# LaurenYTaylor/jsrl-CORL

Measured on AMD Instinct MI355X. Metric: IQL gradient-steps/sec at batch=256 (D4RL obs/act dims), higher is better.
Workload: dtype f32; 1 GPU; IQL step on synthetic buffer (obs=17, act=6, 1000000 rows), batch=256 per GPU; global_batch=256, parallelism=single, prepare_rehearsal_steps=1111

## Files before the change

include/iqlhip.h:

```cpp
#ifndef IQLHIP_H
#define IQLHIP_H

#include <stdint.h>

#ifdef __cplusplus
extern "C" {
#endif

#define IQLHIP_VERSION 400
#define IQLHIP_HIDDEN 256
#define IQLHIP_MAX_INPUT 128
#define IQLHIP_MAX_ACTION 32
#define IQLHIP_MAX_WORLD 8
#define IQLHIP_GRAPH_STEPS 64
#define IQLHIP_N_SCORE 8
#define IQLHIP_N_STATS 16

enum {
  IQLHIP_OK = 0,
  IQLHIP_EINVAL = -1,
  IQLHIP_EHIP = -2,
  IQLHIP_ENOTBOUND = -3,
  IQLHIP_EUNSUPPORTED = -4,
  IQLHIP_EINDEX = -5,
// ... 241 lines not shown
                            void* stream);
int iqlhip_group_train_steps(iqlhip_group* group, const float* const* rows, int64_t ld, const int64_t* size, int32_t B,
                             const void* const* tables, int32_t n, const uint64_t* seeds, const uint64_t* offsets,
                             int32_t flags, void* stream);
int iqlhip_group_train_steps_mixed(iqlhip_group* group, const float* const* rows, int64_t ld, const int64_t* size,
                                   const int32_t* B, const void* const* tables, int32_t n, const uint64_t* seeds,
                                   const uint64_t* offsets, int32_t flags, void* stream);
int iqlhip_group_read_losses(iqlhip_group* group, float* out, int32_t n, void* stream);
int iqlhip_group_read_step_stats(iqlhip_group* group, float* out, int32_t n, void* stream);
int iqlhip_group_online_step(iqlhip_group* group, float* const* rows_dev, int64_t ld, const int64_t* capacity,
                             const int64_t* pointer, const float* row_host, const int64_t* idx_host, int32_t n,
                             const iqlhip_step_scalars* sc, float* out, const float* act_state_host,
                             const int32_t* act_mask, const float* max_action, const uint64_t* act_seed,
                             float* act_out_host, void* stream);
int iqlhip_group_online_step_mixed(iqlhip_group* group, float* const* rows_dev, int64_t ld, const int64_t* capacity,
                                   const int64_t* pointer, const float* row_host, const int64_t* idx_host,
                                   const int32_t* n, const iqlhip_step_scalars* sc, float* out,
                                   const float* act_state_host, const int32_t* act_mask, const float* max_action,
                                   const uint64_t* act_seed, float* act_out_host, void* stream);
int iqlhip_group_online_step_replay2(iqlhip_group* group, float* const* rows_dev, int64_t ld, const int64_t* capacity,
                                     const int64_t* pointer, const float* row_host, const int64_t* idx_host,
                                     const int32_t* n, const iqlhip_step_scalars* sc, float* out,
                                     const float* act_state_host, const int32_t* act_mask, const float* max_action,
                                     const uint64_t* act_seed, float* act_out_host, void* stream,
                                     const float* const* rows_off_dev, const int64_t* size_off, const int32_t* n_off);
int iqlhip_group_train_steps_replay2(iqlhip_group* group, const float* const* rows_off, const int64_t* size_off,
                                     const float* const* rows_on, const int64_t* size_on, int64_t ld, const int32_t* B,
                                     const int32_t* n_off, const void* const* tables, int32_t n, const uint64_t* seeds,
                                     const uint64_t* offsets, void* stream);
int iqlhip_group_train_steps_weighted(iqlhip_group* group, const float* const* rows, int64_t ld, const int64_t* size,
                                      const int32_t* B, const void* const* tables, int32_t n, const uint64_t* seeds,
                                      const uint64_t* offsets, int32_t flags, void* stream,
                                      const iqlhip_weights* const* wtabs);
#define IQLHIP_GROUP_TS_CONTINUE 1
int iqlhip_group_step_rw(iqlhip_group* group, const iqlhip_batch* batches, const iqlhip_step_scalars* sc,
                         const float* const* row_w_dev, float* const* td_out_dev, float* out, void* stream);
int iqlhip_group_train_steps_weighted_is(iqlhip_group* group, const float* const* rows, int64_t ld, const int64_t* size,
                                         const int32_t* B, const void* const* tables, int32_t n, const uint64_t* seeds,
                                         const uint64_t* offsets, int32_t flags, void* stream,
                                         const iqlhip_weights* const* wtabs, const float* is_beta);
int iqlhip_group_train_steps_prioritized(iqlhip_group* group, const float* const* rows, int64_t ld, const int64_t* size,
                                         const int32_t* B, const void* const* tables, int32_t n, const uint64_t* seeds,
                                         const uint64_t* offsets, int32_t flags, void* stream,
                                         iqlhip_weights* const* wtabs, const float* is_beta, const float* alpha,
                                         const float* eps);
#define IQLHIP_GROUP_ACT_WAIT 1
int iqlhip_group_actor_forward(iqlhip_group* group, const float* const* states, int64_t ld_s, const int32_t* rows,
                               const uint64_t* seeds, const float* max_action, float* const* actions, int64_t ld_a,
                               int32_t flags, void* stream);

int iqlhip_group_score_rows(iqlhip_group* group, const float* const* rows_dev, int64_t ld, const int64_t* n_rows,
                            int64_t row0, int64_t n, const int64_t* const* idx_dev, float* const* out_dev,
                            float* spread_dev, int32_t chunk_rows, float* summary , void* stream);

#define IQLHIP_ACT_ROWS 4096
int iqlhip_actor_forward(iqlhip_ctx* ctx, const float* states_dev, int64_t ld_s, int32_t rows, const float* noise_dev,
                         int64_t ld_noise, float max_action, float* actions_dev, int64_t ld_a, void* stream);

int iqlhip_actor_sample(iqlhip_ctx* ctx, const float* states_dev, int64_t ld_s, int32_t rows, uint64_t seed,
                        float max_action, float* actions_dev, int64_t ld_a, void* stream);

int iqlhip_stream_synchronize(void* stream);

typedef struct iqlhip_jsrl iqlhip_jsrl;
int iqlhip_jsrl_create(iqlhip_ctx* const* learners, iqlhip_ctx* const* guides, iqlhip_ctx* const* gates, int k,
                       iqlhip_jsrl** out);
int iqlhip_jsrl_destroy(iqlhip_jsrl* jsrl);
int iqlhip_jsrl_act(iqlhip_jsrl* jsrl, const float* const* states, int64_t ld_s, const int32_t* rows,
                    const int8_t* const* who, const float* gate_max, const uint64_t* seeds,
                    const float* max_action_learner, const float* max_action_guide, float* const* actions, int64_t ld_a,
                    int32_t* const* use_learner, float* const* gate_out, int32_t flags, void* stream);
int iqlhip_jsrl_online_step(iqlhip_jsrl* jsrl, float* rows_dev, int64_t ld, int64_t capacity, int64_t pointer,
                            const float* row_host, const int64_t* idx_host, int32_t n, const iqlhip_step_scalars* sc,
                            float out[3], const float* act_state_host, int8_t who, float gate_max, uint64_t act_seed,
                            float max_action_learner, float max_action_guide, float* act_out_host,
                            int32_t* use_learner_out, float* gate_out, void* stream);

int iqlhip_debug_read(iqlhip_ctx* ctx, const char* name, float* host_out, int64_t max_floats, int64_t* n_out,
                      void* stream);
int iqlhip_debug_time_kernel(iqlhip_ctx* ctx, const iqlhip_batch* batch, int which, int repeat, float* avg_us,
                             void* stream);
int iqlhip_debug_drain_spin(iqlhip_ctx* ctx, void* stream, double* spin_us);
int64_t iqlhip_debug_live_buffers(void);
int iqlhip_set_timing(iqlhip_ctx* ctx, int enabled);
int iqlhip_get_timing(iqlhip_ctx* ctx, float out_us[4]);

typedef struct iqlhip_var iqlhip_var;
typedef struct iqlhip_var_scalars {
  float step_size;
  float bc2_sqrt;
  float beta2, one_minus_beta1, one_minus_beta2, eps;
  int32_t aligned_rewards;
  int32_t reserved;
} iqlhip_var_scalars;
int iqlhip_var_layout(int32_t state_dim, iqlhip_net_layout out[2], int64_t* n_params);
int iqlhip_var_create(int32_t state_dim, int32_t max_rows, int device, iqlhip_var** out);
int iqlhip_var_destroy(iqlhip_var* var);
int iqlhip_var_bind(iqlhip_var* var, float* params, float* exp_avg, float* exp_avg_sq);
int iqlhip_var_step(iqlhip_var* var, const float* batch_dev, int32_t B, int32_t which_net, const iqlhip_var_scalars* sc,
                    void* stream);
int iqlhip_var_values(iqlhip_var* var, const float* batch_dev, int32_t B, int32_t aligned_rewards, float* out_dev,
                      void* stream);
int iqlhip_var_forward_backward(iqlhip_var* var, const float* batch_dev, int32_t B, int32_t which_net,
                                int32_t aligned_rewards, float* grad_out_dev, void* stream);
int iqlhip_var_read_loss(iqlhip_var* var, float* loss, float* head, int32_t n_head, void* stream);

#define IQLHIP_VAR_TRAIN_MAX_STEPS 1024
int iqlhip_var_pack_window(iqlhip_var* var, const float* rows_dev, int64_t ld, int64_t n_rows, int32_t state_dim,
                           int32_t action_dim, int64_t start, int32_t B, float* block_out_dev, void* stream);
int iqlhip_var_values_window(iqlhip_var* var, const float* rows_dev, int64_t ld, int64_t n_rows, int32_t state_dim,
                             int32_t action_dim, int64_t start, int32_t B, int32_t aligned_rewards, float* out_dev,
                             void* stream);
int iqlhip_var_train_steps(iqlhip_var* var, const float* rows_dev, int64_t ld, int64_t size, int32_t action_dim, int32_t B,
                           int32_t n_steps, int32_t which_net, const iqlhip_var_scalars* scalars, uint64_t seed,
                           uint64_t stream_offset, const int64_t* starts_dev, int64_t n_starts, void* stream);
int iqlhip_var_read_train_ring(iqlhip_var* var, float* losses_out, int64_t* starts_out, int32_t n_steps, void* stream);

typedef struct iqlhip_var_group iqlhip_var_group;
int iqlhip_var_group_create(iqlhip_var* const* members, int k, iqlhip_var_group** out);
int iqlhip_var_group_destroy(iqlhip_var_group* group);
int iqlhip_var_group_step(iqlhip_var_group* group, const float* const* blocks_dev, int32_t B, int32_t which_net,
                          const iqlhip_var_scalars* scalars, void* stream);
int iqlhip_var_group_values(iqlhip_var_group* group, const float* const* blocks_dev, int32_t B, const int32_t* aligned_rewards,
                            float* const* outs_dev, void* stream);
int iqlhip_var_group_read_loss(iqlhip_var_group* group, float* losses, float* heads, int32_t n_head, void* stream);
int iqlhip_var_group_pack_windows(iqlhip_var_group* group, const float* const* rows_dev, const int64_t* ld, const int64_t* size,
                                  const int32_t* action_dim, const int64_t* start, int32_t B, float* const* blocks_out_dev,
                                  void* stream);
int iqlhip_var_group_step_windows(iqlhip_var_group* group, const float* const* rows_dev, const int64_t* ld, const int64_t* size,
                                  const int32_t* action_dim, const int64_t* start, int32_t B, int32_t which_net,
                                  const iqlhip_var_scalars* scalars, void* stream);
int iqlhip_var_group_values_windows(iqlhip_var_group* group, const float* const* rows_dev, const int64_t* ld, const int64_t* size,
                                    const int32_t* action_dim, const int64_t* start, int32_t B, const int32_t* aligned_rewards,
                                    float* const* outs_dev, void* stream);
int iqlhip_var_group_train_steps(iqlhip_var_group* group, const float* const* rows_dev, const int64_t* ld, const int64_t* size,
                                 const int32_t* action_dim, int32_t B, int32_t n_steps, int32_t which_net,
                                 const iqlhip_var_scalars* scalars, const uint64_t* seeds, const uint64_t* stream_offsets,
                                 const int64_t* const* starts_dev, const int64_t* n_starts, void* stream);
int iqlhip_var_group_read_train_ring(iqlhip_var_group* group, float* losses_out, int64_t* starts_out, int32_t n_steps,
                                     void* stream);

#ifdef __cplusplus
}
#endif
#endif
```

jsrl-corl_amd/csrc/iqlhip.hip:

```cpp
#include "iqlhip_kernels.h"
#include "iqlhip_lb_kernels.h"
#include "iqlhip_owned.h"

#include <dlfcn.h>

#include <time.h>

#include <algorithm>
#include <cstdarg>
#include <cstdio>
#include <cstdlib>
#include <cstring>
#include <memory>
#include <string>
#include <type_traits>
#include <vector>

#define GRAPH_STEPS IQLHIP_GRAPH_STEPS
static const int kChunkSizes[] = {GRAPH_STEPS, 16, 4, 2, 1};

static thread_local std::string g_err;

static int fail(int code, const char* fmt, ...) {
  char buf[512];
// ... 105 lines not shown
  float* params = nullptr;
  float drop_p = 0.f;
  float inv_batch = 0.f;
  int xch = 0;
  int parity = 0;
  int head = 0;
  int stats = 0;
  int clip = 0;
  ChunkSrc src;
  bool operator==(const GraphKey& o) const {
    return src == o.src && rows == o.rows && ld == o.ld && B == o.B && K == o.K && params == o.params && drop_p == o.drop_p &&
           inv_batch == o.inv_batch && xch == o.xch && parity == o.parity && head == o.head && stats == o.stats && clip == o.clip;
  }
};

struct RcclId { char internal[IQLHIP_UNIQUE_ID_BYTES]; };
struct RcclApi {
  void* lib = nullptr;
  int (*GetUniqueId)(void*) = nullptr;
  int (*CommInitRank)(void**, int, RcclId , int) = nullptr;
  int (*CommDestroy)(void*) = nullptr;
  int (*AllReduce)(const void*, void*, size_t, int, int, void*, hipStream_t) = nullptr;
  const char* (*GetErrorString)(int) = nullptr;
};

struct iqlhip_ctx {
  iqlhip_dims dims;
  iqlhip_hyper hyper;
  iqlhip_layout L;
  int device = 0;
  Owned own;
  float *params = nullptr, *target = nullptr, *m = nullptr, *v = nullptr;
  DevScratch sc{};
  float* flat_tmp = nullptr;
  float* xb = nullptr;
  float* xb2 = nullptr;
  float* xb_act = nullptr;
  float* heads_act = nullptr;
  float* losses_host = nullptr;
  float* on_row_pin = nullptr;
  long long* on_idx_pin = nullptr;
  float* on_loss_pin = nullptr;
  unsigned long long* done_pin = nullptr;
  unsigned long long done_seq = 0;
  float* on_act_pin = nullptr;
  int act_cap = 0;
  unsigned long long act_calls = 0;
  int64_t row_ld = 0;
  unsigned* drop_bits = nullptr;
  float drop_p = 0.f;
  unsigned long long drop_seed = 0, drop_step = 0;
  bool drop_inject = false;
  unsigned* act_drop_bits = nullptr;
  float act_drop_p = 0.f;
  unsigned long long act_drop_seed = 0, act_drop_calls = 0;
  int precision = 0;
  __bf16* wsh = nullptr;
  __bf16* tsh = nullptr;
  float* loss_ring = nullptr;
  int ring_cap = 0;
  iqlhip_step_scalars* sched_cur = nullptr;
  iqlhip_step_scalars* sched_call = nullptr;
  iqlhip_step_scalars* sched_pin[4] = {nullptr, nullptr, nullptr, nullptr};
  unsigned long long* sched_ack = nullptr;
  unsigned long long sched_want[4] = {0, 0, 0, 0};
  unsigned long long call_seq = 0;
  unsigned* setup_arrivals = nullptr;
  bool fwd_lds_set[N_CHUNK_KINDS] = {false, false, false, false, false};
  float* is_buf = nullptr;
  char* prio_buf = nullptr;
  char* prep_save = nullptr;
  hipStream_t sched_stream[4] = {nullptr, nullptr, nullptr, nullptr};
  int sched_slot = 0;
  unsigned long long* hdr = nullptr;
  unsigned long long* stamps = nullptr;
  int k_max = 0;
  int n_chunk_max = 0, n_rt_max = 0;
  size_t lds_fwd = 0, lds_fwd_solo = 0, lds_bwd = 0;
  int n_cus = 256;
  int w0_lds_k = 0;
  int bwd_donate_pct = -1;
  int bwd_spb_force = -1;
  int fwd_spb_force = -1;
  float* pi_t = nullptr;
  __bf16* dh1g = nullptr;
  float* slab_x = nullptr;
  __bf16* wimg = nullptr;
  int lb_enabled = 1;
  int lb_nbb_force = -1, lb_cpb_force = -1, lb_nbi_force = -1;
  bool lb_pi_spread = true;
  bool lb_csplit = true;
  int lb_bwd_part = 0;
  size_t lds_bwd_lb = 0;
  hipStream_t cap_stream = nullptr;
  struct CachedGraph { GraphKey key; hipGraph_t graph; hipGraphExec_t exec; unsigned long long stamp; hipStream_t last;
                       IdleWork* work;
                       hipGraphNode_t setup_node;  };
  struct { bool valid = false; const float* rows = nullptr; int64_t ld = 0, size = 0; int32_t B = 0; uint64_t seed = 0;
           uint64_t next_offset = 0; float drop_p = 0.f; uint64_t drop_seed = 0, drop_step = 0;
           uint64_t wt_gen = 0;
           int cont_class = 0;
           uint64_t wt_ver = 0;
           const void* owner = nullptr;
         } cont;
  std::vector<CachedGraph> graphs;
  unsigned long long graph_clock = 0;
  int xch_mode = IQLHIP_XCH_NONE;
  int rank = 0, world = 1;
  float* xflat = nullptr;
  void* nccl_comm = nullptr;
  char* xblk = nullptr;
  size_t xblk_bytes = 0, xflat_off[2] = {0, 0};
  size_t xslabb_off[2] = {0, 0}, xloss_off[2] = {0, 0};
  long long xslab_b_off[4] = {0, 0, 0, 0};
  char* peer_blk[IQLHIP_MAX_WORLD] = {nullptr, nullptr, nullptr, nullptr, nullptr, nullptr, nullptr, nullptr};
  bool p2p_attached = false;
  unsigned long long* xstatus = nullptr;
  unsigned long long* xstatus_host = nullptr;
  unsigned long long xstep = 0;
  unsigned long long xtimeout_ticks = 500000000ull;
  bool stats_on = false;
  float* stats_part = nullptr;
  int stats_n_part = 0;
  float* stats_last = nullptr;
  float* stats_ring = nullptr;
  float* stats_host = nullptr;
  bool clip_on = false;
  float clip_max[3] = {__builtin_inff(), __builtin_inff(), __builtin_inff()};
  float* clip_dev = nullptr;
  float* clip_host = nullptr;
  hipEvent_t clip_up = nullptr;
  bool clip_up_pending = false;
  float* score_heads = nullptr;
  float* score_pi = nullptr;
  float* score_part = nullptr;
  double* score_acc = nullptr;
  float* score_pin = nullptr;
  unsigned long long* score_status = nullptr;
  bool score_lds_set = false;
  hipStream_t last_stream = nullptr;
  bool has_last_stream = false;
  bool timing = false;
  std::vector<hipEvent_t> ev;
  int ev_used = 0;
  float t_acc[4] = {0, 0, 0, 0};
  int t_n = 0;
};

extern "C" int iqlhip_version(void) { return IQLHIP_VERSION; }
extern "C" const char* iqlhip_last_error(void) { return g_err.c_str(); }

static int check_dims(const iqlhip_dims* d) {
  if (!d) return fail(IQLHIP_EINVAL, "dims is NULL");
  if (d->state_dim < 1 || d->action_dim < 1) return fail(IQLHIP_EINVAL, "state_dim/action_dim must be >= 1");
  if (d->hidden_dim != IQLHIP_HIDDEN || d->n_hidden != 2)
    return fail(IQLHIP_EUNSUPPORTED, "kernels are built for hidden_dim=%d, n_hidden=2 (got %d, %d)", IQLHIP_HIDDEN,
                d->hidden_dim, d->n_hidden);
  if (d->state_dim + d->action_dim > IQLHIP_MAX_INPUT)
    return fail(IQLHIP_EUNSUPPORTED, "state_dim + action_dim > %d", IQLHIP_MAX_INPUT);
  if (d->action_dim > IQLHIP_MAX_ACTION) return fail(IQLHIP_EUNSUPPORTED, "action_dim > %d", IQLHIP_MAX_ACTION);
  if (d->policy != IQLHIP_POLICY_GAUSSIAN && d->policy != IQLHIP_POLICY_DETERMINISTIC)
    return fail(IQLHIP_EINVAL, "unknown policy kind %d", d->policy);
  if (d->max_batch < 1 || d->max_batch > 16384) return fail(IQLHIP_EINVAL, "max_batch must be in [1,16384]");
  return IQLHIP_OK;
}

extern "C" int iqlhip_arena_layout(const iqlhip_dims* d, iqlhip_layout* out) {
  int rc = check_dims(d);
  if (rc) return rc;
  if (!out) return fail(IQLHIP_EINVAL, "out is NULL");
  const int S = d->state_dim, A = d->action_dim, Hd = IQLHIP_HIDDEN;
  int64_t off = 0;
  for (int n = 0; n < 4; ++n) {
    iqlhip_net_layout& nl = out->net[n];
    nl.k_in = (n == IQLHIP_NET_Q1 || n == IQLHIP_NET_Q2) ? S + A : S;
    nl.d_out = (n == IQLHIP_NET_PI) ? A : 1;
    nl.seg_begin = off;
    nl.w1 = off; off += (int64_t)Hd * Hd;
    nl.w0 = off; off += (int64_t)Hd * nl.k_in;
    nl.b0 = off; off += Hd;
    nl.b1 = off; off += Hd;
    nl.w2 = off; off += (int64_t)nl.d_out * Hd;
    nl.b2 = off; off += up(nl.d_out, 4);
    if (n == IQLHIP_NET_PI && d->policy == IQLHIP_POLICY_GAUSSIAN) { nl.log_std = off; off += up(A, 4); }
    else nl.log_std = -1;
    off = up(off, 64);
    nl.seg_end = off;
  }
  out->n_params = off;
  out->target_src = out->net[IQLHIP_NET_Q1].seg_begin;
  out->n_target = out->net[IQLHIP_NET_Q2].seg_end - out->net[IQLHIP_NET_Q1].seg_begin;
  return IQLHIP_OK;
}

extern "C" int64_t iqlhip_row_stride(int32_t S, int32_t A) { return up(2 * (int64_t)S + A + 2, 4); }

static int xld_host(int k0) { int k0p = (k0 + 3) & ~3; return ((k0p + 29) / 32) * 32 + 2; }

extern "C" int iqlhip_destroy(iqlhip_ctx* c);
extern "C" int iqlhip_xch_shutdown(iqlhip_ctx* c);

static int create_impl(iqlhip_ctx* c, const iqlhip_dims* dims, const iqlhip_hyper* hyper, int device) {
  c->dims = *dims;
  c->hyper = *hyper;
  c->device = device;
  iqlhip_arena_layout(dims, &c->L);
  const int MB = dims->max_batch, A = dims->action_dim;
  c->n_chunk_max = (MB + CHUNK_ROWS - 1) / CHUNK_ROWS;
  c->n_rt_max = (MB + RT_ROWS - 1) / RT_ROWS;
  c->sc.max_batch = MB;
  Owned& own = c->own;
  auto dalloc = [&](float** p, size_t nfloat) { return own.dev(p, nfloat * sizeof(float), 0); };
  HIPCHK(dalloc(&c->sc.h0, (size_t)4 * MB * HID));
  HIPCHK(dalloc(&c->sc.h1, (size_t)4 * MB * HID));
  HIPCHK(dalloc(&c->sc.heads, (size_t)MB * HEAD_LD + (size_t)NSPLIT * MB * A));
  c->row_ld = iqlhip_row_stride(dims->state_dim, A);
  HIPCHK(dalloc(&c->xb, (size_t)MB * c->row_ld));
  HIPCHK(dalloc(&c->xb2, (size_t)MB * c->row_ld));
  HIPCHK(own.pin(&c->losses_host, 4 * sizeof(float)));
  HIPCHK(own.pin(&c->on_row_pin, (size_t)c->row_ld * sizeof(float)));
  HIPCHK(own.pin(&c->on_idx_pin, (size_t)MB * sizeof(long long)));
  HIPCHK(own.pin(&c->on_loss_pin, 4 * sizeof(float)));
  HIPCHK(own.pin(&c->done_pin, 8 * sizeof(unsigned long long), true));
  HIPCHK(own.pin(&c->on_act_pin, (size_t)(IQLHIP_MAX_INPUT + IQLHIP_MAX_ACTION) * sizeof(float)));
  c->act_cap = std::max(MB, IQLHIP_ACT_ROWS);
  HIPCHK(dalloc(&c->xb_act, (size_t)c->act_cap * c->row_ld));
  HIPCHK(dalloc(&c->heads_act, (size_t)c->act_cap * A * NSPLIT));
  HIPCHK(own.dev(&c->drop_bits, (size_t)4 * MB * 8 * sizeof(unsigned), 0xFF));
  HIPCHK(dalloc(&c->sc.slab_a, (size_t)c->n_chunk_max * c->L.n_params));
  size_t sb = 0;
  for (int n = 0; n < 4; ++n) {
    c->sc.slab_b_off[n] = (long long)sb;
    sb += (size_t)c->n_rt_max * ((size_t)HID * c->L.net[n].k_in + HID);
  }
  HIPCHK(dalloc(&c->sc.slab_b, sb));
  HIPCHK(dalloc(&c->sc.loss_parts, 2 * 4 * 64));
  HIPCHK(dalloc(&c->pi_t, (size_t)MB * 65));
  HIPCHK(dalloc(&c->sc.losses, 4));
  HIPCHK(dalloc(&c->flat_tmp, (size_t)c->L.n_params + 4));
  c->k_max = 1024;
  c->ring_cap = c->k_max;
  HIPCHK(own.pin(&c->loss_ring, (size_t)c->ring_cap * 4 * sizeof(float), true));
  HIPCHK(own.dev(&c->sched_cur, (size_t)GRAPH_STEPS * sizeof(iqlhip_step_scalars)));
  HIPCHK(own.dev(&c->sched_call, (size_t)c->k_max * sizeof(iqlhip_step_scalars)));
  for (int i = 0; i < 4; ++i) HIPCHK(own.pin(&c->sched_pin[i], (size_t)c->k_max * sizeof(iqlhip_step_scalars)));
  HIPCHK(own.pin(&c->sched_ack, 8 * sizeof(unsigned long long), true));
  HIPCHK(own.dev(&c->setup_arrivals, 64, 0));
  HIPCHK(own.dev(&c->hdr, HDR_WORDS * sizeof(unsigned long long), 0));
  HIPCHK(own.dev(&c->xstatus, 2 * sizeof(unsigned long long), 0));
  HIPCHK(own.pin(&c->xstatus_host, 2 * sizeof(unsigned long long), true));
  HIPCHK(dalloc(&c->xflat, (size_t)up(c->L.n_params + 4, 64)));
  HIPCHK(hipStreamCreateWithFlags(&c->cap_stream, hipStreamNonBlocking));
#ifdef IQL_STAMPS
  HIPCHK(own.dev(&c->stamps, 4096 * 16 * sizeof(unsigned long long), 0));
#endif
  const int kq = dims->state_dim + dims->action_dim;
  const int ks_ = dims->state_dim;
  const size_t fwd_fixed = (size_t)(RT_ROWS * H0_LD + RT_ROWS * T64_LD + RT_ROWS * (int)c->row_ld +
                                    (((A + 15) & ~15) * W2_LD + 32) + 512 + 16) * sizeof(float);
  auto fits = [&](int k) { return fwd_fixed + (size_t)HID * k * sizeof(float) + 4096 <= (size_t)160 * 1024 - 1024; };
  int w0_lds_k = 0;
  if (kq <= W0_DMA_MAX_K && fits(kq)) w0_lds_k = kq;
  else if (ks_ <= W0_DMA_MAX_K && fits(ks_)) w0_lds_k = ks_;
  if (const char* ov = getenv("IQLHIP_W0_LDS_K")) w0_lds_k = std::min(w0_lds_k, atoi(ov));
  c->w0_lds_k = w0_lds_k;
  if (const char* ov = getenv("IQLHIP_BWD_DONATE_PCT")) c->bwd_donate_pct = std::max(0, std::min(100, atoi(ov)));
  if (const char* ov = getenv("IQLHIP_BWD_SPB_L2")) c->bwd_spb_force = std::max(0, std::min(2, atoi(ov)));
  if (const char* ov = getenv("IQLHIP_FWD_SPB_L2")) c->fwd_spb_force = std::max(0, std::min(2, atoi(ov)));
  if (const char* ov = getenv("IQLHIP_LB")) c->lb_enabled = atoi(ov) != 0;
  if (const char* ov = getenv("IQLHIP_LB_NBB")) c->lb_nbb_force = std::max(2, atoi(ov));
  if (const char* ov = getenv("IQLHIP_LB_CSPLIT")) c->lb_csplit = atoi(ov) != 0;
  if (const char* ov = getenv("IQLHIP_LB_PI_SPREAD")) c->lb_pi_spread = atoi(ov) != 0;
  if (const char* ov = getenv("IQLHIP_LB_CPB")) c->lb_cpb_force = std::max(1, atoi(ov));
  if (const char* ov = getenv("IQLHIP_LB_NBI")) c->lb_nbi_force = std::max(2, atoi(ov));
  c->lds_fwd = fwd_fixed + (size_t)HID * w0_lds_k * sizeof(float) + (w0_lds_k > W0_LDS_MAX_K ? 4096 : 0);
  c->lds_fwd_solo = std::max(c->lds_fwd, (size_t)(81 * 1024));
  {
    int ncu = 0;
    if (hipDeviceGetAttribute(&ncu, hipDeviceAttributeMultiprocessorCount, c->device) == hipSuccess && ncu > 0) c->n_cus = ncu;
  }
  const int dyld = ((A + 15) & ~15) + 4;
  const size_t lds_a = (size_t)(4 * 32 * T64_LD + 2 * CHUNK_ROWS * dyld + 32 * 32 + 64 + CHUNK_ROWS) * sizeof(float);
  const size_t lds_b = (size_t)(RT_ROWS * H0_LD + 4 * 32 * T64_LD + RT_ROWS * T64_LD + RT_ROWS * 36 + 4 +
                                RT_ROWS * XR_LD_MAX) * sizeof(float);
  c->lds_bwd = std::max(lds_a, lds_b);
  c->lds_bwd_lb = (size_t)(3 * 32 * H0B_LD + 32 * LB_DYLD) * 2 + 32 * 4 + (size_t)(2 * 4 * 32 + 16) * 4;
  int rc = set_max_lds(3, c->lds_fwd_solo, [](unsigned m) { return fwd_kernel(m & 1, m & 2, m & 4); });
  if (!rc) rc = set_max_lds(2, c->lds_fwd_solo, [](unsigned m) { return fwd_one_kernel(m & 1, m & 2); });
  if (!rc) rc = set_max_lds(3, c->lds_bwd, [](unsigned m) { return bwd_kernel(m & 1, m & 2, m & 4); });
  if (!rc) rc = set_max_lds(1, c->lds_bwd_lb, [](unsigned m) { return bwd_rows_kernel(m & 1); });
  if (!rc) rc = set_max_lds(2, c->lds_bwd, [](unsigned m) { return bwd_rw_kernel(m & 1, m & 2); });
  c->fwd_lds_set[(int)ChunkKind::Plain] = !rc;
  return rc;
}

extern "C" int iqlhip_create(const iqlhip_dims* dims, const iqlhip_hyper* hyper, int device, iqlhip_ctx** out) {
  int rc = check_dims(dims);
  if (rc) return rc;
  if (!hyper || !out) return fail(IQLHIP_EINVAL, "hyper/out is NULL");
  int ndev = 0;
  HIPCHK(hipGetDeviceCount(&ndev));
  if (device < 0 || device >= ndev) return fail(IQLHIP_EHIP, "device %d not available (%d visible)", device, ndev);
  DevGuard guard(device);
  iqlhip_ctx* c = new iqlhip_ctx();
  rc = create_impl(c, dims, hyper, device);
  if (rc) {
    const std::string msg = g_err;
    iqlhip_destroy(c);
    g_err = msg;
    return rc;
  }
  *out = c;
  return IQLHIP_OK;
}

static void free_graph(iqlhip_ctx::CachedGraph& g) {
  if (g.exec) (void)hipGraphExecDestroy(g.exec);
  if (g.graph) (void)hipGraphDestroy(g.graph);
  if (g.work) (void)hipFree(g.work);
}
static void drop_graph(iqlhip_ctx* c) {
  for (auto& g : c->graphs) {
    if (g.last) (void)hipStreamSynchronize(g.last);
    free_graph(g);
  }
  c->graphs.clear();
  c->cont.valid = false;
}

extern "C" int iqlhip_destroy(iqlhip_ctx* c) {
  if (!c) return IQLHIP_OK;
  DevGuard guard(c->device);
  (void)hipDeviceSynchronize();
  drop_graph(c);
  (void)iqlhip_xch_shutdown(c);
  for (hipEvent_t e : c->ev) (void)hipEventDestroy(e);
  if (c->cap_stream) (void)hipStreamDestroy(c->cap_stream);
  c->own.release_all();
  delete c;
  return IQLHIP_OK;
}

extern "C" int iqlhip_set_hyper(iqlhip_ctx* c, const iqlhip_hyper* h) {
  if (!c || !h) return fail(IQLHIP_EINVAL, "NULL argument");
  c->hyper = *h;
  drop_graph(c);
  return IQLHIP_OK;
}

extern "C" int iqlhip_set_precision(iqlhip_ctx* c, int mode) {
  if (!c) return fail(IQLHIP_EINVAL, "NULL ctx");
  if (mode != 0 && mode != 1) return fail(IQLHIP_EINVAL, "precision mode must be 0 (f32) or 1 (bf16 operands)");
  if (mode != c->precision) drop_graph(c);
  if (mode == 1 && !c->wsh) {
    DevGuard guard(c->device);
    const int rc = all_or_nothing(c->own, [&]() -> int {
      Owned& own = c->own;
      HIPCHK(own.dev(&c->wsh, (size_t)up(c->L.n_params, 64) * sizeof(__bf16)));
      HIPCHK(own.dev(&c->tsh, (size_t)up(c->L.n_target, 64) * sizeof(__bf16)));
      const size_t MB = (size_t)c->dims.max_batch;
      HIPCHK(own.dev(&c->dh1g, (8 * MB * HID + MB * 32 + MB * LB_XLD + 4 * 65536 + 8192) * sizeof(__bf16), 0));
      HIPCHK(own.dev(&c->wimg, (size_t)6 * IMG_STRIDE * sizeof(__bf16), 0));
      HIPCHK(own.dev(&c->slab_x, (size_t)64 * c->L.n_params * sizeof(float), 0));
      return IQLHIP_OK;
    });
    if (rc) return rc;
  }
  c->precision = mode;
  return IQLHIP_OK;
}

extern "C" int iqlhip_get_counters(const iqlhip_ctx* c, uint64_t out[2]) {
  if (!c || !out) return fail(IQLHIP_EINVAL, "NULL argument");
  out[0] = c->drop_step;
  out[1] = c->act_calls;
// ... 192 lines not shown
  p.hy = c->hyper;
  p.sc = c->sc;
  p.xb = c->xb;
  p.ld = (int)c->row_ld;
  p.rows = rows;
  p.S = S;
  p.A = A;
  p.policy = c->dims.policy;
  p.inv_batch = inv_batch;
  p.n_params = L.n_params;
  p.drop_bits = (c->drop_p > 0.f) ? c->drop_bits : nullptr;
  p.drop_scale = (c->drop_p > 0.f) ? 1.f / (1.f - c->drop_p) : 1.f;
  p.only_inst = -1;
  p.w0_lds_k = c->w0_lds_k;
  p.g_work = nullptr;
  return p;
}

static StepParams act_step_params(const iqlhip_ctx* c, int rows) {
  StepParams p = make_step(c, rows, 1.f / (float)rows);
  p.xb = c->xb_act;
  p.only_inst = 6;
  p.slot[6] = -1;
  p.drop_bits = nullptr;
  p.drop_scale = 1.f;
  p.sc.heads = c->heads_act;
  p.sc.max_batch = 0;
  if (c->act_drop_p > 0.f) {
    p.drop_bits = c->act_drop_bits;
    p.drop_scale = 1.f / (1.f - c->act_drop_p);
    p.sc.max_batch = c->act_cap;
    p.sc.heads = c->heads_act - (size_t)c->act_cap * HEAD_LD;
  }
  return p;
}

static UpdParams make_upd(const iqlhip_ctx* c, const iqlhip_step_scalars* sc, int rows, const float* flat) {
  UpdParams u;
  u.L = c->L;
  u.sc = *sc;
  u.tau = c->hyper.tau;
  u.one_minus_tau = c->hyper.one_minus_tau;
  u.params = c->params; u.target = c->target; u.m = c->m; u.v = c->v;
  u.slab_a = c->sc.slab_a; u.slab_b = c->sc.slab_b;
  for (int n = 0; n < 4; ++n) u.slab_b_off[n] = c->sc.slab_b_off[n];
  u.flat_grads = flat;
  u.loss_parts = c->sc.loss_parts;
  u.losses = c->sc.losses;
  u.losses_mirror = nullptr;
  u.loss_ring = nullptr;
  u.ring_slot = 0;
  u.n_chunk = (rows + CHUNK_ROWS - 1) / CHUNK_ROWS;
  u.n_rt = (rows + RT_ROWS - 1) / RT_ROWS;
  u.n_loss = u.n_chunk;
  u.slab_x = nullptr;
  u.n_x = 0;
  if (use_lb(c, rows)) {
    const LbGeom gm = lb_geom(c, rows);
    u.n_chunk = gm.n_cg;
    u.slab_x = c->slab_x;
    u.n_x = gm.nbb;
    u.loss_parts = c->sc.loss_parts + 256;
    u.n_loss = 1;
  }
  u.batch_rows = rows;
  u.sched = nullptr;
  u.sched_idx = 0;
  u.ring_hdr = nullptr;
  u.adv_hdr = nullptr; u.adv_k = 0; u.adv_rows = 0;
  u.done_flag = nullptr; u.done_val = 0;
  u.wsh = (c->precision == 1) ? c->wsh : nullptr;
  u.tsh = (c->precision == 1) ? c->tsh : nullptr;
  u.wimg = (c->precision == 1 && use_lb(c, rows)) ? c->wimg : nullptr;
  if (getenv("IQLHIP_LB_NOIMG")) u.wimg = nullptr;
  u.n_peer = 0;
  u.peer_direct = 0;
  for (int r = 0; r < IQLHIP_MAX_WORLD; ++r) { u.peer_flat[r] = nullptr; u.peer_slab_b[r] = nullptr; u.peer_loss[r] = nullptr; }
  return u;
}

static size_t fwd_lds(const iqlhip_ctx* c, int n_blocks) { return (n_blocks <= c->n_cus) ? c->lds_fwd_solo : c->lds_fwd; }

static const void* fwd_kernel_of(ChunkKind kind, bool bf, bool dma, bool multi);
static void launch_fwd_grid(const iqlhip_ctx* c, const StepParams& p, int nb, hipStream_t st, ChunkKind kind = ChunkKind::Plain) {
  const bool dma = c->w0_lds_k > W0_LDS_MAX_K;
  const bool bf = c->precision == 1, multi = (p.spb_l2 & 3) > 0;
  const void* kernel = (p.only_inst >= 0) ? (const void*)fwd_one_kernel(bf, dma) : fwd_kernel_of(kind, bf, dma, multi);
  void* args[] = {const_cast<StepParams*>(&p)};
  (void)hipLaunchKernel(kernel, dim3(nb), dim3(256), args, fwd_lds(c, nb), st);
}
static int ensure_fwd_lds(iqlhip_ctx* c, ChunkKind kind) {
  if (c->fwd_lds_set[(int)kind]) return IQLHIP_OK;
  DevGuard guard(c->device);
  if (int rc = set_max_lds(3, c->lds_fwd_solo, [kind](unsigned m) { return fwd_kernel_of(kind, m & 1, m & 2, m & 4); })) return rc;
  c->fwd_lds_set[(int)kind] = true;
  return IQLHIP_OK;
}

static int fwd_spb_l2(const iqlhip_ctx* c, int n_rt) {
  if (c->fwd_spb_force >= 0) return c->fwd_spb_force;
  if (8 * n_rt * NSPLIT <= c->n_cus) return 0;
  if (8 * n_rt * 2 <= c->n_cus) return 1;
  return 2;
}
static int fwd_blocks(int n_rt, int l2) { return (l2 == 2) ? 8 * 2 * ((n_rt + 1) / 2) : 8 * n_rt * (NSPLIT >> l2); }
static void launch_fwd(const iqlhip_ctx* c, const StepParams& p_in, hipStream_t st, ChunkKind kind = ChunkKind::Plain) {
  StepParams p = p_in;
  if (p.only_inst < 0 && use_lb(c, p.rows)) {
    const LbArgs a = lb_args(c, p.rows);
    const int kq = c->dims.state_dim + c->dims.action_dim;
    const dim3 grid(8 * a.nbi);
    const bool spread = a.n_rt > 2 * a.nbi && c->lb_pi_spread;
    if (spread) {
      if (kq <= 32) hipLaunchKernelGGL((iql_fwd_lb_kernel<1, true>), grid, dim3(256), 0, st, p, a);
      else if (kq <= 64) hipLaunchKernelGGL((iql_fwd_lb_kernel<2, true>), grid, dim3(256), 0, st, p, a);
      else hipLaunchKernelGGL((iql_fwd_lb_kernel<3, true>), grid, dim3(256), 0, st, p, a);
    } else {
      if (kq <= 32) hipLaunchKernelGGL((iql_fwd_lb_kernel<1, false>), grid, dim3(256), 0, st, p, a);
      else if (kq <= 64) hipLaunchKernelGGL((iql_fwd_lb_kernel<2, false>), grid, dim3(256), 0, st, p, a);
      else hipLaunchKernelGGL((iql_fwd_lb_kernel<3, false>), grid, dim3(256), 0, st, p, a);
    }
    return;
  }
  const int n_rt = (p.rows + RT_ROWS - 1) / RT_ROWS;
  p.spb_l2 = fwd_spb_l2(c, n_rt);
  launch_fwd_grid(c, p, fwd_blocks(n_rt, p.spb_l2), st, kind);
}
static int bwd_spb_l2(const iqlhip_ctx* c, int n_chunk, int n_rt) {
  if (c->bwd_spb_force >= 0) return c->bwd_spb_force;
  return (4 * (32 * n_chunk + 4 * n_rt) <= 2 * c->n_cus) ? 0 : 2;
}
static int bwd_blocks(int n_chunk, int n_rt, int l2, int n_don) {
  const int per_net = 32 * n_chunk + (4 >> l2) * n_rt;
  return 8 * ((per_net + 1) / 2 + (n_don + 5) / 6);
}
struct BwdWords { const float *heads, *xb, *h1, *h0, *params; unsigned dims, ldB, mbc, rts; };
static BwdWords bwd_words(const iqlhip_ctx* c, const StepParams& p, int n_chunk, int n_rt, unsigned spb_l2) {
  BwdWords w;
  w.heads = p.sc.heads; w.xb = p.xb; w.h1 = p.sc.h1; w.h0 = p.sc.h0; w.params = c->params;
  w.dims = (unsigned)p.S | ((unsigned)p.A << 8) | ((unsigned)p.policy << 14);
  w.ldB = (unsigned)p.ld | ((unsigned)p.rows << 10);
  w.mbc = (unsigned)p.sc.max_batch | ((unsigned)n_chunk << 16);
  w.rts = (unsigned)n_rt | (spb_l2 << 10);
  return w;
}
struct RowWeights { const float* w; float* td; };
static void launch_bwd(const iqlhip_ctx* c, const StepParams& p_in, hipStream_t st, const RowWeights* rw = nullptr) {
  StepParams p = p_in;
  if (use_lb(c, p.rows)) {
    const LbArgs a = lb_args(c, p.rows);
    const int kq = c->dims.state_dim + c->dims.action_dim;
    (void)kq;
    if (c->lb_bwd_part != 2) {
      const bool csplit = lb_geom(c, p.rows).csplit;
      hipLaunchKernelGGL(bwd_rows_kernel(csplit), dim3(8 * (csplit ? a.nbb : a.nbb / 2)), dim3(256), c->lds_bwd_lb, st, p, a);
    }
    if (c->lb_bwd_part != 1)
      hipLaunchKernelGGL(iql_bwd_gemm_kernel, dim3(8 * ((LB_NJOB * a.n_cg + 1 + 1) / 2)), dim3(256), 0, st, p, a);
    return;
  }
  const int n_rt = (p.rows + RT_ROWS - 1) / RT_ROWS;
  const int n_chunk = (p.rows + CHUNK_ROWS - 1) / CHUNK_ROWS;
  int l2 = bwd_spb_l2(c, n_chunk, n_rt);
  if (c->precision == 1 && l2 > 0) l2 = 2;
  int n_don = 0;
  if (l2 > 0) {
    const int pct = (c->bwd_donate_pct >= 0) ? c->bwd_donate_pct : std::max(30, std::min(50, 22 + c->dims.action_dim));
    n_don = std::min(32 * n_chunk, (32 * n_chunk * pct + 50) / 100);
  }
// ... 4702 lines not shown
```

jsrl-corl_amd/csrc/iqlhip_fwd_body.inc:

```
  RT_ENTRY();
  const int bid = blockIdx.x;
  const int fx = bid & 7, fh = fx >> 2, fr = bid >> 3;
  constexpr unsigned FWD_PAIR_A = 0x6541u, FWD_PAIR_B = 0x7320u;
  const int inst = ONE ? p.only_inst : (int)((((fr & 1) ? FWD_PAIR_B : FWD_PAIR_A) >> (4 * (fx & 3))) & 7u);
  if (inst >= 7) {
    if (p.g_work) idle_block_work<MIXED_IDLE>(p.g_work, (fr >> 1) * 2 + fh, (int)(gridDim.x >> 3));
    return;
  }
  const int spb_l2 = MULTI ? (p.spb_l2 & 3) : 0;
  const int spb = 1 << spb_l2;
  int ns, rt;
  if (ONE) {
    ns = bid & (NSPLIT - 1);
    rt = bid >> 2;
  } else if (spb_l2 == 0) {
    ns = 2 * ((fr >> 1) & 1) + fh;
    rt = fr >> 2;
    if (ROW_EXIT && rt * RT_ROWS >= p.rows) return;
  } else if (spb_l2 == 1) {
    ns = 2 * fh;
    rt = fr >> 1;
    if (ROW_EXIT && rt * RT_ROWS >= p.rows) return;
  } else {
    ns = 0;
    rt = 2 * (fr >> 1) + fh;
    if (rt * RT_ROWS >= p.rows) return;
  }
  const int row0 = rt * RT_ROWS;
  const int tid = threadIdx.x, lane = tid & 63, wave = tid >> 6;
  const int l15 = lane & 15, g = lane >> 4;

  const NetPtrs np = p.inst[inst];
  const int xoff = p.xoff[inst];
  const int slot = p.slot[inst];
  const int k0 = np.k0;
  const int k0p = (k0 + 3) & ~3;
  const int D = np.d;
  const int ld = p.ld;
  const int B = p.rows;
  const int w0k = p.w0_lds_k;
  const float* xb = p.xb;
  float* h0g = p.sc.h0;
  float* h1g = p.sc.h1;
  float* headsg = p.sc.heads;
  const int MB = p.sc.max_batch;
  const int Aact = p.A;
  PIN_P(np.w0); PIN_P(np.b0); PIN_P(np.w1); PIN_P(np.b1); PIN_P(np.w2); PIN_P(np.b2);
  PIN_S(k0); PIN_S(D); PIN_S(xoff); PIN_S(slot); PIN_S(ld); PIN_S(B); PIN_S(MB); PIN_S(Aact);
  PIN_P(xb); PIN_P(h0g); PIN_P(h1g); PIN_P(headsg); PIN_S(w0k);
  const bool w0_lds = W0DMA ? (k0 <= w0k) : (k0 <= min(w0k, W0_LDS_MAX_K));
  const bool w0_dma = W0DMA && w0_lds && (k0 > W0_LDS_MAX_K);

  extern __shared__ __attribute__((aligned(16))) float smem[];
  float* H0s = smem;
  float* H1s = H0s + RT_ROWS * H0_LD;
  float* Xr = H1s + RT_ROWS * T64_LD;
  float* W2s = Xr + RT_ROWS * ld;
  const int w2s_words = ((Aact + 15) & ~15) * W2_LD + 32;
  unsigned* Mk = (unsigned*)(W2s + w2s_words);
  float* W0s = W2s + w2s_words + 512;

  STAMP_BASE(p, 0);
  STAMP(p, 0);
  const int n_x = RT_ROWS * ld / 4;
  const int x_last = B * ld / 4 - 1;
  f32x4 xr[XR_MAX_F4];
  xr_load(xr, xb, row0 * ld / 4, n_x, x_last);
  f32x4 w2pre[2];
#pragma unroll
  for (int q = 0; q < 2; ++q) {
    const int e = min(tid + 256 * q, D * 16 - 1);
    w2pre[q] = *(const f32x4*)(np.w2 + (unsigned)((e >> 4) * HID + ns * 64 + 4 * (e & 15)));
  }
  const float b2v = np.b2[min(tid, D - 1)];
  f32x4 bias0[4];
#pragma unroll
  for (int ct = 0; ct < 4; ++ct) bias0[ct] = *(const f32x4*)(np.b0 + (unsigned)(wave * 64 + ct * 16 + 4 * g));
  f32x4 bias1 = *(const f32x4*)(np.b1 + (unsigned)(ns * 64 + wave * 16 + 4 * g));
  const bool drop = (inst == 6) && (p.drop_bits != nullptr);
  unsigned mk0 = 0xFFFFFFFFu, mk1 = 0xFFFFFFFFu;
  if (drop) {
    const int mrow = min(row0 + (tid >> 3), B - 1);
    mk0 = p.drop_bits[mrow * 8 + (tid & 7)];
    mk1 = p.drop_bits[(MB + mrow) * 8 + (tid & 7)];
  }
  const int n_w0v = 64 * k0;
  f32x4 w0v[16];
  if (w0_dma) {
    const int nj = (n_w0v + 255) >> 8;
    for (int j = 0; j < nj; ++j)
      lds_dma16(np.w0 + 4 * min(tid + 256 * j, n_w0v - 1), W0s + 4 * (256 * j + 64 * wave));
  } else if (w0_lds) {
#pragma unroll
    for (int j = 0; j < 8; ++j) w0v[j] = *(const f32x4*)(np.w0 + 4u * (unsigned)min(tid + 256 * j, n_w0v - 1));
    if (k0 > 32) {
#pragma unroll
      for (int j = 8; j < 16; ++j) w0v[j] = *(const f32x4*)(np.w0 + 4u * (unsigned)min(tid + 256 * j, n_w0v - 1));
    }
  }
  int n1 = ns * 64 + wave * 16 + l15;
  f32x4 bw[BF16 ? 1 : 16];
  bf16x8 bwb[BF16 ? 8 : 1];
  __bf16* H0b = (__bf16*)H0s;

  xr_store(xr, Xr, n_x);
  const int Dp = (D + 15) & ~15;
#pragma unroll
  for (int q = 0; q < 2; ++q) {
    const int e = tid + 256 * q;
    if (e < Dp * 16) *(f32x4*)(W2s + (e >> 4) * W2_LD + 4 * (e & 15)) = (e < D * 16) ? w2pre[q] : (f32x4){0.f, 0.f, 0.f, 0.f};
  }
  if (tid < D) W2s[Dp * W2_LD + tid] = b2v;
  Mk[tid] = mk0;
  Mk[256 + tid] = mk1;
  if (w0_lds && !w0_dma) {
#pragma unroll
    for (int j = 0; j < 8; ++j) {
      const int f = tid + 256 * j;
      if (f < n_w0v) *(f32x4*)(W0s + 4 * f) = w0v[j];
    }
    if (k0 > 32) {
#pragma unroll
      for (int j = 8; j < 16; ++j) {
        const int f = tid + 256 * j;
        if (f < n_w0v) *(f32x4*)(W0s + 4 * f) = w0v[j];
      }
    }
  }
  __syncthreads();
  const bool bw_in_l0 = !BF16 && w0_lds;
#define BW_LOAD(ks_) bw[ks_] = *(const f32x4*)(np.w1 + (unsigned)(n1 * HID + 16 * (ks_) + 4 * g))
#define BWB_AT(unit_, j_) (*(const bf16x8*)((const __bf16*)np.w1 + (unsigned)((unit_) * HID + 32 * (j_) + 8 * g)))
  if constexpr (BF16) {
#pragma unroll
    for (int j = 0; j < 8; ++j) bwb[j] = BWB_AT(n1, j);
  } else if (!bw_in_l0) {
#pragma unroll
    for (int ks = 0; ks < 16; ++ks) BW_LOAD(ks);
  }
  STAMP(p, 1);

  {
    f32x4 acc[2][4];
#pragma unroll
    for (int i = 0; i < 2; ++i)
#pragma unroll
      for (int j = 0; j < 4; ++j) acc[i][j] = (f32x4){0.f, 0.f, 0.f, 0.f};
    const int nks = k0p >> 2;
    const float* x0 = Xr + l15 * ld + xoff;
    const float* x1 = Xr + (16 + l15) * ld + xoff;
    float bcur[4], bnxt[4], acur[2], anxt[2];
    if (w0_lds && nks <= 8) {
      const float* wl[4];
#pragma unroll
      for (int ct = 0; ct < 4; ++ct) wl[ct] = W0s + (wave * 64 + ct * 16 + l15) * k0;
      float bq[8][4], aq[8][2];
#pragma unroll
      for (int ks = 0; ks < 8; ++ks) {
        const int kk = 4 * ks + g;
        const int kc = min(kk, k0 - 1);
#pragma unroll
        for (int ct = 0; ct < 4; ++ct) bq[ks][ct] = wl[ct][kc];
        const float xa = x0[kc], xb_ = x1[kc];
        aq[ks][0] = (kk < k0) ? xa : 0.f;
        aq[ks][1] = (kk < k0) ? xb_ : 0.f;
      }
#pragma unroll
      for (int ks = 0; ks < 8; ++ks) {
        asm volatile("" : "+v"(aq[ks][0]), "+v"(aq[ks][1]));
      }
      STAMP(p, 5);
      if constexpr (BF16) {
        l0_chunk_bf16(acc, bq, aq);
      } else {
#pragma unroll
        for (int ks = 0; ks < 8; ++ks) {
          if (ks < nks) {
#pragma unroll
            for (int ct = 0; ct < 4; ++ct) {
              acc[0][ct] = MFMA16(bq[ks][ct], aq[ks][0], acc[0][ct]);
              acc[1][ct] = MFMA16(bq[ks][ct], aq[ks][1], acc[1][ct]);
            }
          }
          if (ks < 4) {
#pragma unroll
            for (int k2 = 4 * ks; k2 < 4 * ks + 4; ++k2) BW_LOAD(k2);
          }
        }
      }
      STAMP(p, 6);
    } else if (w0_lds) {
      const float* wl[4];
#pragma unroll
      for (int ct = 0; ct < 4; ++ct) wl[ct] = W0s + (wave * 64 + ct * 16 + l15) * k0;
      float bqA[8][4], aqA[8][2], bqB[8][4], aqB[8][2];
      auto rd = [&](float (&bq)[8][4], float (&aq)[8][2], const int base) {
#pragma unroll
        for (int h = 0; h < 2; ++h) {
          if (base + 4 * h < nks) {
#pragma unroll
            for (int k4 = 0; k4 < 4; ++k4) {
              const int ks = 4 * h + k4;
              const int kk = 4 * (base + ks) + g;
              const int kc = min(kk, k0 - 1);
#pragma unroll
              for (int ct = 0; ct < 4; ++ct) bq[ks][ct] = wl[ct][kc];
              const float xa = x0[kc], xb_ = x1[kc];
              aq[ks][0] = (kk < k0) ? xa : 0.f;
              aq[ks][1] = (kk < k0) ? xb_ : 0.f;
            }
#pragma unroll
            for (int k4 = 0; k4 < 4; ++k4) asm volatile("" : "+v"(aq[4 * h + k4][0]), "+v"(aq[4 * h + k4][1]));
          } else if (BF16) {
#pragma unroll
            for (int k4 = 0; k4 < 4; ++k4) {
              aq[4 * h + k4][0] = 0.f;
              aq[4 * h + k4][1] = 0.f;
#pragma unroll
              for (int ct = 0; ct < 4; ++ct) bq[4 * h + k4][ct] = 0.f;
            }
          }
        }
      };
      auto mm = [&](const float (&bq)[8][4], const float (&aq)[8][2], const int base) {
        if constexpr (BF16) {
          l0_chunk_bf16(acc, bq, aq);
        } else {
#pragma unroll
          for (int ks = 0; ks < 8; ++ks) {
            if (base + ks < nks) {
#pragma unroll
              for (int ct = 0; ct < 4; ++ct) {
                acc[0][ct] = MFMA16(bq[ks][ct], aq[ks][0], acc[0][ct]);
                acc[1][ct] = MFMA16(bq[ks][ct], aq[ks][1], acc[1][ct]);
              }
            }
            if (base == 0) {
              BW_LOAD(2 * ks);
              BW_LOAD(2 * ks + 1);
            }
          }
        }
      };
      rd(bqA, aqA, 0);
      rd(bqB, aqB, 8);
      STAMP(p, 5);
      mm(bqA, aqA, 0);
      if (nks > 16) rd(bqA, aqA, 16);
      mm(bqB, aqB, 8);
      if (nks > 16) mm(bqA, aqA, 16);
      STAMP(p, 6);
    } else {
      const float* wrow[4];
#pragma unroll
      for (int ct = 0; ct < 4; ++ct) wrow[ct] = np.w0 + (wave * 64 + ct * 16 + l15) * k0;
#pragma unroll
      for (int ct = 0; ct < 4; ++ct) { const float v = wrow[ct][min(g, k0 - 1)]; bcur[ct] = (g < k0) ? v : 0.f; }
      for (int ks = 0; ks < nks; ++ks) {
        const int kn = 4 * (ks + 1) + g;
#pragma unroll
        for (int ct = 0; ct < 4; ++ct) { const float v = wrow[ct][min(kn, k0 - 1)]; bnxt[ct] = (kn < k0) ? v : 0.f; }
        const int kc = min(4 * ks + g, k0 - 1);
        const float a0 = x0[kc];
        const float a1 = x1[kc];
#pragma unroll
        for (int ct = 0; ct < 4; ++ct) {
          acc[0][ct] = MFMA16(bcur[ct], a0, acc[0][ct]);
          acc[1][ct] = MFMA16(bcur[ct], a1, acc[1][ct]);
        }
#pragma unroll
        for (int ct = 0; ct < 4; ++ct) bcur[ct] = bnxt[ct];
      }
    }
#pragma unroll
    for (int ct = 0; ct < 4; ++ct) {
#pragma unroll
      for (int rtile = 0; rtile < 2; ++rtile) {
        f32x4 h;
#pragma unroll
        for (int reg = 0; reg < 4; ++reg) h[reg] = fmaxf(acc[rtile][ct][reg] + bias0[ct][reg], 0.f);
        if (drop) {
          const unsigned bits = Mk[(rtile * 16 + l15) * 8 + wave * 2 + (ct >> 1)] >> ((ct & 1) * 16 + 4 * g);
#pragma unroll
          for (int reg = 0; reg < 4; ++reg) h[reg] = ((bits >> reg) & 1u) ? h[reg] * p.drop_scale : 0.f;
        }
        if constexpr (BF16) {
          bf16x4 hb_;
#pragma unroll
          for (int reg = 0; reg < 4; ++reg) hb_[reg] = (__bf16)h[reg];
          *(bf16x4*)(H0b + (rtile * 16 + l15) * H0B_LD + wave * 64 + ct * 16 + 4 * g) = hb_;
        } else {
          *(f32x4*)(H0s + (rtile * 16 + l15) * H0_LD + wave * 64 + ct * 16 + 4 * g) = h;
        }
      }
    }
  }
  STAMP(p, 7);
  __syncthreads();
  STAMP(p, 2);

  for (int it = 0;; ++it) {
  const bool more = MULTI && (it + 1 < spb);
  f32x4 bias1n = bias1;
  if (more) {
#pragma unroll
    for (int q = 0; q < 2; ++q) {
      const int e = min(tid + 256 * q, D * 16 - 1);
      w2pre[q] = *(const f32x4*)(np.w2 + (unsigned)((e >> 4) * HID + (ns + 1) * 64 + 4 * (e & 15)));
    }
    bias1n = *(const f32x4*)(np.b1 + (unsigned)((ns + 1) * 64 + wave * 16 + 4 * g));
  }
  if (slot >= 0) {
    const int rl = tid >> 3;
    const int row = row0 + rl;
    if (row < B) {
#pragma unroll
      for (int j = 0; j < 2; ++j) {
        const int col = ns * 64 + 4 * ((tid & 7) + 8 * j);
        if constexpr (BF16)
          *(bf16x4*)((__bf16*)h0g + (unsigned)((slot * MB + row) * HID + col)) = *(const bf16x4*)(H0b + rl * H0B_LD + col);
        else
          *(f32x4*)(h0g + (unsigned)((slot * MB + row) * HID + col)) = *(const f32x4*)(H0s + rl * H0_LD + col);
      }
    }
  }

  if (it == 0) STAMP(p, 8);
  {
    f32x4 acc0 = (f32x4){0.f, 0.f, 0.f, 0.f}, acc1 = acc0;
    if constexpr (BF16) {
      bf16x8 b0[8], b1[8];
#pragma unroll
      for (int j = 0; j < 8; ++j) {
        b0[j] = *(const bf16x8*)(H0b + l15 * H0B_LD + 32 * j + 8 * g);
        b1[j] = *(const bf16x8*)(H0b + (16 + l15) * H0B_LD + 32 * j + 8 * g);
      }
#pragma unroll
      for (int j = 0; j < 8; ++j) {
        acc0 = MFMA_BF16(bwb[j], b0[j], acc0);
        acc1 = MFMA_BF16(bwb[j], b1[j], acc1);
        if ((j & 1) && more) {
          bwb[j - 1] = BWB_AT(n1 + 64, j - 1);
          bwb[j] = BWB_AT(n1 + 64, j);
        }
      }
    } else {
#pragma unroll
      for (int ks = 0; ks < 16; ++ks) {
        const f32x4 a0 = *(const f32x4*)(H0s + l15 * H0_LD + 16 * ks + 4 * g);
        const f32x4 a1 = *(const f32x4*)(H0s + (16 + l15) * H0_LD + 16 * ks + 4 * g);
#pragma unroll
        for (int t = 0; t < 4; ++t) {
          acc0 = MFMA16(bw[ks][t], a0[t], acc0);
          acc1 = MFMA16(bw[ks][t], a1[t], acc1);
        }
        if ((ks & 3) == 3 && more) {
#pragma unroll
          for (int k2 = ks - 3; k2 <= ks; ++k2)
            bw[k2] = *(const f32x4*)(np.w1 + (unsigned)((n1 + 64) * HID + 16 * k2 + 4 * g));
        }
      }
    }
    if (it == 0) STAMP(p, 9);
    f32x4 h0, h1;
#pragma unroll
    for (int reg = 0; reg < 4; ++reg) {
      h0[reg] = fmaxf(acc0[reg] + bias1[reg], 0.f);
      h1[reg] = fmaxf(acc1[reg] + bias1[reg], 0.f);
    }
    if (drop) {
      const int word = ns * 2 + (wave >> 1), sh = (wave & 1) * 16 + 4 * g;
      const unsigned ba = Mk[256 + l15 * 8 + word] >> sh, bb_ = Mk[256 + (16 + l15) * 8 + word] >> sh;
#pragma unroll
      for (int reg = 0; reg < 4; ++reg) {
        h0[reg] = ((ba >> reg) & 1u) ? h0[reg] * p.drop_scale : 0.f;
        h1[reg] = ((bb_ >> reg) & 1u) ? h1[reg] * p.drop_scale : 0.f;
      }
    }
    *(f32x4*)(H1s + l15 * T64_LD + wave * 16 + 4 * g) = h0;
    *(f32x4*)(H1s + (16 + l15) * T64_LD + wave * 16 + 4 * g) = h1;
  }
  if (it == 0) STAMP(p, 10);
// ... 72 lines not shown
```

jsrl-corl_amd/csrc/iqlhip_isweight_kernels.h:

```cpp
#pragma once

__device__ __forceinline__ float is_weight(float q, float q_min, float beta) {
  return __builtin_amdgcn_exp2f(beta * __builtin_amdgcn_logf(q_min / q));
}

__device__ __forceinline__ unsigned long long wt_leaf(const WTab& wt, unsigned i) {
  return wt.tab[i] - (((wt.local ? (i & 63u) : i) != 0u) ? wt.tab[i - 1u] : 0ull);
}

__global__ __launch_bounds__(256) void iql_draw_indices_weighted_q_kernel(long long* idx, float* qf, long long n_idx, WTab wt,
                                                                          unsigned long long seed, unsigned long long offset) {
  const long long wave = __builtin_amdgcn_readfirstlane((int)(blockIdx.x * 4u + (threadIdx.x >> 6)));
  const long long n_waves = (long long)gridDim.x * 4;
  for (long long j0 = wave; j0 < n_idx; j0 += 2 * n_waves) {
    const long long j1 = j0 + n_waves;
    const unsigned long long j[2] = {(unsigned long long)j0, (unsigned long long)(j1 < n_idx ? j1 : j0)};
    long long i[2];
    draw_index_weighted<2>(wt, seed, offset, j, i);
    if ((threadIdx.x & 63) == 0) {
      idx[j0] = i[0];
      qf[j0] = (float)wt_leaf(wt, (unsigned)i[0]);
      if (j1 < n_idx) {
        idx[j1] = i[1];
        qf[j1] = (float)wt_leaf(wt, (unsigned)i[1]);
      }
    }
  }
}

__global__ __launch_bounds__(256) void iql_is_weights_kernel(float* c, long long n, long long group, float beta) {
  __shared__ float red[4];
  const long long lo = (long long)blockIdx.x * group, hi = min(lo + group, n);
  float m = __builtin_inff();
  for (long long j = lo + threadIdx.x; j < hi; j += 256) m = fminf(m, c[j]);
#pragma unroll
  for (int o = 32; o > 0; o >>= 1) m = fminf(m, __shfl_xor(m, o));
  if ((threadIdx.x & 63) == 0) red[threadIdx.x >> 6] = m;
  __syncthreads();
  const float q_min = fminf(fminf(red[0], red[1]), fminf(red[2], red[3]));
  for (long long j = lo + threadIdx.x; j < hi; j += 256) c[j] = is_weight(c[j], q_min, beta);
}

__device__ __forceinline__ void gather_rows_drawn_weighted_q(const float* rows, long long ld, float* xb, float* qf, int n,
                                                             const WTab& wt, unsigned long long seed, unsigned long long ctr0,
                                                             unsigned long long j0, int wave, int n_waves) {
  const int q = (int)(ld >> 2);
  const int lane = (int)(threadIdx.x & 63);
  for (int r0 = wave; r0 < n; r0 += 2 * n_waves) {
    const int r1 = r0 + n_waves;
    const bool two = r1 < n;
    const unsigned long long j[2] = {j0 + (unsigned long long)r0, j0 + (unsigned long long)(two ? r1 : r0)};
    long long i[2];
    draw_index_weighted<2>(wt, seed, ctr0, j, i);
    if (lane == 0) {
      qf[r0] = (float)wt_leaf(wt, (unsigned)i[0]);
      if (two) qf[r1] = (float)wt_leaf(wt, (unsigned)i[1]);
    }
    for (int c4 = lane; c4 < q; c4 += 64) {
      const f32x4 a = *(const f32x4*)(rows + i[0] * ld + 4 * c4);
      f32x4 b = a;
      if (two) b = *(const f32x4*)(rows + i[1] * ld + 4 * c4);
      *(f32x4*)(xb + (long long)r0 * ld + 4 * c4) = a;
      if (two) *(f32x4*)(xb + (long long)r1 * ld + 4 * c4) = b;
    }
  }
}
__device__ __forceinline__ void idle_gather_weighted_q(const IdleWork& w, unsigned long long seed, unsigned long long ctr0,
                                                       unsigned long long j0, int blk, int nblk) {
  const WTab wt = w.wt;
  const int wave = __builtin_amdgcn_readfirstlane(blk * 4 + (int)(threadIdx.x >> 6));
  gather_rows_drawn_weighted_q(w.rows, w.ld, w.xb_dst, w.q_dst, w.n, wt, seed, ctr0, j0, wave, nblk * 4);
}
__device__ __forceinline__ void idle_is_weights(const IdleWork& w) {
  if (threadIdx.x < 64) {
    const float beta = *w.is_beta;
    float m = __builtin_inff();
    for (int r = (int)threadIdx.x; r < w.n; r += 64) m = fminf(m, w.q_src[r]);
#pragma unroll
    for (int o = 32; o > 0; o >>= 1) m = fminf(m, __shfl_xor(m, o));
    for (int r = (int)threadIdx.x; r < w.n; r += 64) w.c_dst[r] = is_weight(w.q_src[r], m, beta);
  }
}

__global__ __launch_bounds__(256) void iql_call_setup_weighted_is_kernel(unsigned long long* hdr, ChunkHdr h,
                                                                         iqlhip_step_scalars* sched_call,
                                                                         const iqlhip_step_scalars* sched_src, int n_steps,
                                                                         const float* rows, long long ld, float* xb, int B,
                                                                         unsigned* drop_dst, int drop_words, unsigned drop_thresh,
                                                                         unsigned* arrivals, unsigned long long* ack,
                                                                         unsigned long long ack_val, WTab wt, float* q_dst,
                                                                         float* beta_dev, float beta) {
  call_setup_head(hdr, h, sched_call, sched_src, n_steps, arrivals, ack, ack_val);
  if (blockIdx.x == 0 && threadIdx.x == 0) *beta_dev = beta;
  if (B > 0)
    gather_rows_drawn_weighted_q(rows, ld, xb, q_dst, B, wt, h.w[HDR_SEED], h.w[HDR_OFFSET], h.w[HDR_POS],
                                 __builtin_amdgcn_readfirstlane((int)(blockIdx.x * 4u + (threadIdx.x >> 6))), (int)gridDim.x * 4);
  if (drop_dst)
    dropmask_words(drop_dst, drop_words, drop_thresh, h.w[HDR_DROP_SEED], h.w[HDR_DROP_STEP],
                   ((int)gridDim.x - 1 - (int)blockIdx.x) * 256 + (int)threadIdx.x, (int)gridDim.x * 256);
}

template <bool W0DMA, bool MULTI>
__global__ __launch_bounds__(256) __attribute__((amdgpu_waves_per_eu(2))) void iql_fwd_weighted_is_kernel(StepParams p) {
  constexpr bool BF16 = false, ONE = false, ROW_EXIT = false;
  constexpr int MIXED_IDLE = 3;
#include "iqlhip_fwd_body.inc"
}
```

jsrl-corl_amd/csrc/iqlhip_kernels.h:

```cpp
#pragma once
#include <hip/hip_runtime.h>
#include <stdint.h>
#include "iqlhip.h"

typedef float f32x4 __attribute__((ext_vector_type(4)));
typedef float f32x2 __attribute__((ext_vector_type(2)));
typedef float f32x4u __attribute__((ext_vector_type(4), aligned(4)));

#define HID 256
#define RT_ROWS 32
#define CHUNK_ROWS 256
#define H0_LD 260
#define H0B_LD 264
#define T64_LD 68
#define NSPLIT 4
#define HEAD_LD 24
#define W0_LDS_MAX_K 64
#define W0_DMA_MAX_K 96
#define W2_LD 68

#define MFMA16(a, b, c) __builtin_amdgcn_mfma_f32_16x16x4f32((a), (b), (c), 0, 0, 0)

typedef __bf16 bf16x8 __attribute__((ext_vector_type(8)));
#define MFMA_BF16(a, b, c) __builtin_amdgcn_mfma_f32_16x16x32_bf16((a), (b), (c), 0, 0, 0)
// ... 38 lines not shown
}

struct DevScratch {
  float* h0;
  float* h1;
  float* heads;
  float* slab_a;
  float* slab_b;
  float* loss_parts;
  float* losses;
  long long slab_b_off[4];
  int max_batch;
};

#ifdef IQL_STAMPS
__device__ __forceinline__ unsigned long long iql_memtime() {
  unsigned long long t;
  __builtin_amdgcn_sched_barrier(0);
  asm volatile("s_memtime %0\n\ts_waitcnt lgkmcnt(0)" : "=s"(t) :: "memory");
  __builtin_amdgcn_sched_barrier(0);
  return t;
}
#define STAMP(p, i)                                                                        \
  do {                                                                                     \
    const unsigned long long t_ = iql_memtime();                                           \
    if (stamps_ && threadIdx.x == 0 && blockIdx.x < stamps_blocks_) stamps_[(long long)blockIdx.x * 16 + (i)] = t_; \
  } while (0)
#define STAMP_BASE(p, off) unsigned long long* const stamps_ = (p).stamps ? (p).stamps + (off) : nullptr; \
  const unsigned stamps_blocks_ = (unsigned)((4096 * 16 - (off)) / 16)
__device__ __forceinline__ unsigned long long iql_realtime() {
  unsigned long long t;
  __builtin_amdgcn_sched_barrier(0);
  asm volatile("s_memrealtime %0\n\ts_waitcnt lgkmcnt(0)" : "=s"(t) :: "memory");
  __builtin_amdgcn_sched_barrier(0);
  return t;
}
#define RT_ENTRY() const unsigned long long rt_entry_ = iql_realtime()
#define RT_STAMP(p, i, t)                                                                  \
  do {                                                                                     \
    if (stamps_ && threadIdx.x == 0 && blockIdx.x < stamps_blocks_) stamps_[(long long)blockIdx.x * 16 + (i)] = (t); \
  } while (0)
#else
#define STAMP(p, i) do {} while (0)
#define STAMP_BASE(p, off) do {} while (0)
#define RT_ENTRY() do {} while (0)
#define RT_STAMP(p, i, t) do {} while (0)
#define iql_realtime() 0ull
#define rt_entry_ 0ull
#endif

struct NetPtrs {
  const float *w0, *b0, *w1, *b1, *w2, *b2;
  int k0, d;
};
struct NetGrad {
  long long w1, b1, w2, b2, log_std;
};

struct StepParams {
  unsigned long long* stamps;
  NetPtrs inst[8];
  int xoff[8];
  int slot[8];
  NetPtrs net[4];
  NetGrad go[4];
  const float* log_std;
  iqlhip_hyper hy;
  DevScratch sc;
  const float* xb;
  int ld, rows;
  int S, A, policy;
  float inv_batch;
  long long n_params;
  const unsigned* drop_bits;
  float drop_scale;
  int only_inst;
  int w0_lds_k;
  int spb_l2;
  const struct IdleWork* g_work;
};

#define PIN_S(x) asm volatile("" ::"s"(x))
#define PIN_P(x) asm volatile("" ::"s"((unsigned long long)(uintptr_t)(x)))

#define XR_MAX_F4 9
#define XR_LD_MAX 260
template <int Q0, int Q1>
__device__ __forceinline__ void xr_issue(f32x4 (&xr)[XR_MAX_F4], const float* xb, int first_f4, int n_x, int x_last) {
#pragma unroll
  for (int q = Q0; q < Q1; ++q) {
    const int f = min(first_f4 + min((int)threadIdx.x + 256 * q, n_x - 1), x_last);
    xr[q] = *(const f32x4*)(xb + 4u * (unsigned)f);
  }
}
__device__ __forceinline__ void xr_load(f32x4 (&xr)[XR_MAX_F4], const float* xb, int first_f4, int n_x, int x_last) {
#pragma unroll
  for (int q = 0; q < XR_MAX_F4; ++q) xr[q] = (f32x4){0.f, 0.f, 0.f, 0.f};
  xr_issue<0, 3>(xr, xb, first_f4, n_x, x_last);
  if (n_x > 3 * 256) {
    xr_issue<3, 5>(xr, xb, first_f4, n_x, x_last);
    if (n_x > 5 * 256) xr_issue<5, 9>(xr, xb, first_f4, n_x, x_last);
  }
}
__device__ __forceinline__ void xr_store(const f32x4 (&xr)[XR_MAX_F4], float* Xr, int n_x) {
#pragma unroll
  for (int q = 0; q < XR_MAX_F4; ++q) {
    const int f = (int)threadIdx.x + 256 * q;
    if (f < n_x) *(f32x4*)(Xr + 4 * f) = xr[q];
  }
}

__device__ __forceinline__ void lds_dma16(const float* gsrc, float* lds_wave_base) {
  __builtin_amdgcn_global_load_lds((const __attribute__((address_space(1))) void*)gsrc,
                                   (__attribute__((address_space(3))) void*)lds_wave_base, 16, 0, 0);
}

__device__ __forceinline__ void gather_rows_flat(const float* rows, long long ld, const long long* idx, float* xb,
                                                 int n, int first, int stride, long long n_rows = 0) {
  const int q = (int)(ld >> 2);
  const int total = n * q;
  for (int e = first; e < total; e += stride) {
    const int r = e / q, c4 = e - r * q;
    const long long i = idx[r];
    f32x4 v;
    if (n_rows > 0 && (i < 0 || i >= n_rows)) {
      const float nanv = __builtin_nanf("");
      v = (f32x4){nanv, nanv, nanv, nanv};
    } else {
      v = *(const f32x4*)(rows + i * ld + 4 * c4);
    }
    *(f32x4*)(xb + (long long)r * ld + 4 * c4) = v;
  }
}

enum { HDR_SIZE = 0, HDR_SEED = 1, HDR_OFFSET = 2, HDR_DROP_STEP = 3, HDR_DROP_SEED = 4, HDR_BASE = 5, HDR_XSTEP = 6,
       HDR_POS = 7, HDR_SIZE_ON = 8, HDR_WORDS = 9 };
struct ChunkHdr { unsigned long long w[HDR_WORDS]; };

__device__ __forceinline__ void philox4x32_10(uint32_t c[4], uint32_t k0, uint32_t k1) {
#pragma unroll
  for (int r = 0; r < 10; ++r) {
    const uint64_t p0 = (uint64_t)0xD2511F53u * c[0];
    const uint64_t p1 = (uint64_t)0xCD9E8D57u * c[2];
    const uint32_t n0 = (uint32_t)(p1 >> 32) ^ c[1] ^ k0;
    const uint32_t n1 = (uint32_t)p1;
    const uint32_t n2 = (uint32_t)(p0 >> 32) ^ c[3] ^ k1;
    const uint32_t n3 = (uint32_t)p0;
    c[0] = n0; c[1] = n1; c[2] = n2; c[3] = n3;
    k0 += 0x9E3779B9u; k1 += 0xBB67AE85u;
  }
}

__device__ __forceinline__ unsigned keep_word(uint32_t w, uint32_t tag, unsigned thresh, unsigned long long seed,
                                              unsigned long long pos) {
  unsigned word = 0;
#pragma unroll
  for (int j = 0; j < 8; ++j) {
    uint32_t c[4] = {w, (uint32_t)j | tag, (uint32_t)pos, (uint32_t)(pos >> 32)};
    philox4x32_10(c, (uint32_t)seed, (uint32_t)(seed >> 32));
#pragma unroll
    for (int q = 0; q < 4; ++q) word |= (c[q] >= thresh ? 1u : 0u) << (4 * j + q);
  }
  return word;
}
__device__ __forceinline__ void dropmask_words(unsigned* bits, int n_words, unsigned thresh, unsigned long long seed,
                                               unsigned long long step, int first, int stride) {
// ... 21 lines not shown
    *(f32x4*)(xb + (long long)r * ld + 4 * c4) = *(const f32x4*)(rows + i * ld + 4 * c4);
  }
}

__device__ __forceinline__ void gather_rows_drawn2(const float* rows_off, const float* rows_on, long long ld, float* xb, int n,
                                                   int n_off, unsigned long long seed, unsigned long long ctr0,
                                                   unsigned long long j0, unsigned long long size_off,
                                                   unsigned long long size_on, int first, int stride) {
  const int q = (int)(ld >> 2);
  const int total = n * q;
  for (int e = first; e < total; e += stride) {
    const int r = e / q, c4 = e - r * q;
    const bool on = r >= n_off;
    const long long i = draw_index(seed, ctr0, j0 + (unsigned long long)r, on ? size_on : size_off);
    const float* src = on ? rows_on : rows_off;
    *(f32x4*)(xb + (long long)r * ld + 4 * c4) = *(const f32x4*)(src + i * ld + 4 * c4);
  }
}

struct WTab {
  const unsigned long long* tab;
  unsigned n;
  unsigned short levels;
  unsigned short local;
};
static_assert(sizeof(WTab) == 16, "WTab keeps its size: it lies inside IdleWork and among kernel arguments");

struct IdleWork {
  const float* rows;
  long long ld;
  float* xb_dst;
  const unsigned long long* hdr;
  const iqlhip_step_scalars* sched_call;
  iqlhip_step_scalars* sched_dst;
  unsigned* drop_dst;
  int drop_words;
  unsigned drop_thresh;
  int n;
  int k;
  const float* rows_on;
  int n_off;
  WTab wt;
  float* q_dst;
  const float* q_src;
  float* c_dst;
  const float* is_beta;
  long long* idx_dst;
};
__device__ __forceinline__ void idle_gather_weighted(const IdleWork& w, unsigned long long seed, unsigned long long ctr0,
                                                     unsigned long long j0, int blk, int nblk);
__device__ __forceinline__ void idle_gather_weighted_q(const IdleWork& w, unsigned long long seed, unsigned long long ctr0,
                                                       unsigned long long j0, int blk, int nblk);
__device__ __forceinline__ void idle_is_weights(const IdleWork& w);
__device__ __forceinline__ void idle_gather_weighted_qi(const IdleWork& w, unsigned long long seed, unsigned long long ctr0,
                                                        unsigned long long j0, int blk, int nblk);
template <int MODE = 0>
__device__ __forceinline__ void idle_block_work(const IdleWork* wk, int blk, int nblk) {
  constexpr bool MIXED = MODE == 1;
  const IdleWork w = *wk;
  const unsigned long long size = w.hdr[HDR_SIZE], seed = w.hdr[HDR_SEED], ctr0 = w.hdr[HDR_OFFSET], pos = w.hdr[HDR_POS];
  const unsigned long long base = w.hdr[HDR_BASE], dseed = w.hdr[HDR_DROP_SEED], dstep = w.hdr[HDR_DROP_STEP];
  if constexpr (MODE == 4) {
    idle_gather_weighted_qi(w, seed, ctr0, pos + (unsigned long long)(w.k + 1) * (unsigned long long)w.n, blk, nblk);
    if (blk == nblk - 1) idle_is_weights(w);
  } else if constexpr (MODE == 3) {
    idle_gather_weighted_q(w, seed, ctr0, pos + (unsigned long long)(w.k + 1) * (unsigned long long)w.n, blk, nblk);
    if (blk == nblk - 1) idle_is_weights(w);
  } else if constexpr (MODE == 2)
    idle_gather_weighted(w, seed, ctr0, pos + (unsigned long long)(w.k + 1) * (unsigned long long)w.n, blk, nblk);
  else if (MIXED)
    gather_rows_drawn2(w.rows, w.rows_on, w.ld, w.xb_dst, w.n, w.n_off, seed, ctr0,
                       pos + (unsigned long long)(w.k + 1) * (unsigned long long)w.n, size, w.hdr[HDR_SIZE_ON],
                       blk * 256 + (int)threadIdx.x, nblk * 256);
  else
    gather_rows_drawn(w.rows, w.ld, w.xb_dst, w.n, seed, ctr0, pos + (unsigned long long)(w.k + 1) * (unsigned long long)w.n,
                      size, blk * 256 + (int)threadIdx.x, nblk * 256);
  if (blk == nblk - 1 && threadIdx.x < sizeof(iqlhip_step_scalars) / sizeof(float))
    ((float*)w.sched_dst)[threadIdx.x] = ((const float*)(w.sched_call + base + (unsigned long long)w.k))[threadIdx.x];
  if (w.drop_dst)
    dropmask_words(w.drop_dst, w.drop_words, w.drop_thresh, dseed, dstep + (unsigned long long)(w.k + 1),
                   (nblk - 1 - blk) * 256 + (int)threadIdx.x, nblk * 256);
}

__device__ __forceinline__ void l0_chunk_bf16(f32x4 (&acc)[2][4], const float (&bq)[8][4], const float (&aq)[8][2]) {
  bf16x8 B[2];
#pragma unroll
  for (int r = 0; r < 2; ++r) {
    float t8[8];
#pragma unroll
    for (int e = 0; e < 8; ++e) t8[e] = aq[e][r];
    B[r] = pack8s(t8);
  }
#pragma unroll
  for (int ct = 0; ct < 4; ++ct) {
    float t8[8];
#pragma unroll
    for (int e = 0; e < 8; ++e) t8[e] = bq[e][ct];
    const bf16x8 A = pack8s(t8);
    acc[0][ct] = MFMA_BF16(A, B[0], acc[0][ct]);
    acc[1][ct] = MFMA_BF16(A, B[1], acc[1][ct]);
  }
}

template <bool BF16, bool W0DMA, bool MULTI, bool ONE = false>
__global__ __launch_bounds__(256) __attribute__((amdgpu_waves_per_eu(2))) void iql_fwd_kernel(StepParams p) {
  constexpr bool ROW_EXIT = false;
  constexpr bool MIXED_IDLE = false;
#include "iqlhip_fwd_body.inc"
}

struct RowIn {
  f32x4 h[6];
  float r, d;
};

__device__ __forceinline__ void row_issue(const StepParams& p, int row, RowIn& in) {
  const float* hb = p.sc.heads;
  const unsigned o = (unsigned)row * (unsigned)HEAD_LD;
#pragma unroll
  for (int i = 0; i < 6; ++i) in.h[i] = *(const f32x4*)(hb + (o + 4u * i));
  const float* xb = p.xb;
  const unsigned ox = (unsigned)row * (unsigned)p.ld + (unsigned)(2 * p.S + p.A);
  in.r = xb[ox];
  in.d = xb[ox + 1u];
}

__device__ __forceinline__ void row_issue_hot(const float* heads, const float* xb, int ld, int S, int A, int row, RowIn& in) {
  const unsigned o = (unsigned)row * (unsigned)HEAD_LD;
#pragma unroll
  for (int i = 0; i < 6; ++i) in.h[i] = *(const f32x4*)(heads + (o + 4u * i));
  const unsigned ox = (unsigned)row * (unsigned)ld + (unsigned)(2 * S + A);
  in.r = xb[ox];
  in.d = xb[ox + 1u];
}

__device__ __forceinline__ float sum4(const f32x4 v) { return ((v[0] + v[1]) + v[2]) + v[3]; }

__device__ __forceinline__ float tanh_via_exp(float x) {
  const float e = __builtin_amdgcn_exp2f(x * 2.885390081777927f);
  return 1.f - 2.f * __builtin_amdgcn_rcpf(e + 1.f);
}

struct PiConst { float ls, ivar; };
__device__ __forceinline__ float pi_ls_issue(const StepParams& p) {
  const float* src = (p.policy == IQLHIP_POLICY_GAUSSIAN) ? p.log_std : p.xb;
  return src[min((int)(threadIdx.x & 63), p.A - 1)];
}
__device__ __forceinline__ float pi_ls_issue_hot(const float* log_std, const float* xb, int policy, int A) {
  const float* src = (policy == IQLHIP_POLICY_GAUSSIAN) ? log_std : xb;
  return src[min((int)(threadIdx.x & 63), A - 1)];
}
__device__ __forceinline__ PiConst pi_consts_hot(const StepParams& p, int policy, int net, float lsr) {
  PiConst c;
  c.ls = 0.f;
  c.ivar = 1.f;
  if (net == IQLHIP_NET_PI && policy == IQLHIP_POLICY_GAUSSIAN) {
    c.ls = fminf(fmaxf(lsr, p.hy.log_std_min), p.hy.log_std_max);
    const float sig = expf(c.ls);
    c.ivar = 1.f / (sig * sig);
  }
  return c;
}
__device__ __forceinline__ PiConst pi_consts(const StepParams& p, int net, float lsr) {
  PiConst c;
  c.ls = 0.f;
  c.ivar = 1.f;
  if (net == IQLHIP_NET_PI && p.policy == IQLHIP_POLICY_GAUSSIAN) {
    c.ls = fminf(fmaxf(lsr, p.hy.log_std_min), p.hy.log_std_max);
    const float sig = expf(c.ls);
    c.ivar = 1.f / (sig * sig);
  }
  return c;
}

__device__ __forceinline__ void row_finish(const StepParams& p, int net, const RowIn& in, float* dyrow,
                                           float& lossA, float& lossB) {
  const float invB = p.inv_batch;
  lossA = 0.f;
  lossB = 0.f;
  if (net == IQLHIP_NET_V) {
    const float tq = fminf(sum4(in.h[2]), sum4(in.h[3]));
    const float u = tq - sum4(in.h[1]);
    const float wgt = fabsf(p.hy.iql_tau - ((u < 0.f) ? 1.f : 0.f));
    lossA = wgt * u * u;
    dyrow[0] = (-2.f * wgt * u) * invB;
    return;
  }
  const float nv = sum4(in.h[0]);
  const float y = in.r + ((1.f - in.d) * p.hy.discount) * nv;
  const float e1 = sum4(in.h[4]) - y;
  const float e2 = sum4(in.h[5]) - y;
  lossA = e1 * e1;
  lossB = e2 * e2;
  dyrow[0] = ((net == IQLHIP_NET_Q1) ? e1 : e2) * invB;
}
__device__ __forceinline__ f32x2 row_td_errors(const StepParams& p, const RowIn& in) {
  const float nv = sum4(in.h[0]);
  const float y = in.r + ((1.f - in.d) * p.hy.discount) * nv;
  return (f32x2){sum4(in.h[4]) - y, sum4(in.h[5]) - y};
}

__device__ __forceinline__ float block_sum_256(float v, float* red ) {
#pragma unroll
  for (int o = 32; o > 0; o >>= 1) v += __shfl_xor(v, o);
  __syncthreads();
  if ((threadIdx.x & 63) == 0) red[threadIdx.x >> 6] = v;
  __syncthreads();
  return (red[0] + red[1]) + (red[2] + red[3]);
}

template <int NK>
__device__ __forceinline__ void dh1_mfma(f32x4 (&pre)[4][2], const float* dYs, const float* W2s, int DYA, int wave,
                                         int g, int l15) {
#pragma unroll
  for (int k1 = 0; k1 < NK; ++k1) {
    float a1[4];
#pragma unroll
    for (int t = 0; t < 4; ++t) a1[t] = dYs[(64 * wave + 16 * t + l15) * DYA + 4 * k1 + g];
    const f32x2 b1 = *(const f32x2*)(W2s + (4 * k1 + g) * 32 + 2 * l15);
#pragma unroll
    for (int t = 0; t < 4; ++t) {
      pre[t][0] = MFMA16(a1[t], b1[0], pre[t][0]);
      pre[t][1] = MFMA16(a1[t], b1[1], pre[t][1]);
    }
  }
}

__device__ __forceinline__ void pi_items8(const f32x4 (&hv)[8], const float (&acv)[8], const float (&wv)[8], bool live,
                                          bool gauss, float ivar, float ls, float invB, float (&dyv)[8], float (&dlv)[8],
                                          float& lossA) {
#pragma unroll
  for (int cc = 0; cc < 8; ++cc) {
    const float w = wv[cc];
    const float mu = tanh_via_exp(sum4(hv[cc]));
    const float diff = acv[cc] - mu;
    const float q = diff * diff * ivar;
    const float l_g = w * (0.5f * q + ls + 0.918938533204672742f);
    const float l_d = w * (diff * diff);
    const float dmu_g = (-(w * diff) * ivar) * invB;
    const float dmu_d = (-2.f * w * diff) * invB;
    const float dmu = gauss ? dmu_g : dmu_d;
    lossA += live ? (gauss ? l_g : l_d) : 0.f;
    dyv[cc] = live ? dmu * (1.f - mu * mu) : 0.f;
    dlv[cc] = (live && gauss) ? w * (1.f - q) : 0.f;
  }
}

#define BROW(r) (FULL ? (r) : min((r), B - 1))
struct ArenaOff { unsigned w0, b0, b1, w2, b2, log_std; int k0, d; };
__device__ __forceinline__ ArenaOff arena_off(int net, int S, int A, bool gauss) {
  auto seg = [&](int k, int d, bool ls) -> unsigned {
    const unsigned n = 65536u + 256u * (unsigned)k + 512u + 256u * (unsigned)d + (((unsigned)d + 3u) & ~3u) + (ls ? (((unsigned)A + 3u) & ~3u) : 0u);
    return (n + 63u) & ~63u;
  };
  const unsigned sV = seg(S, 1, false), sQ = seg(S + A, 1, false);
  const unsigned begin = (net == IQLHIP_NET_V) ? 0u : ((net == IQLHIP_NET_Q1) ? sV : ((net == IQLHIP_NET_Q2) ? sV + sQ : sV + 2u * sQ));
  ArenaOff o;
  o.k0 = (net == IQLHIP_NET_Q1 || net == IQLHIP_NET_Q2) ? S + A : S;
  o.d = (net == IQLHIP_NET_PI) ? A : 1;
  o.w0 = begin + 65536u;
  o.b0 = o.w0 + 256u * (unsigned)o.k0;
  o.b1 = o.b0 + 256u;
  o.w2 = o.b1 + 256u;
  o.b2 = o.w2 + 256u * (unsigned)o.d;
  o.log_std = o.b2 + (((unsigned)o.d + 3u) & ~3u);
  return o;
}
template <bool BF16, bool FULL, bool MULTI>
__global__ __launch_bounds__(256) void iql_bwd_kernel(const float* q_heads, const float* q_xb, const float* q_h1, const float* q_h0,
                                                      const float* q_params, unsigned q_dims, unsigned q_ldB, unsigned q_mbc,
                                                      unsigned q_rts, StepParams p) {
  constexpr bool KPF = true;
  constexpr bool RW = false;
  const float* const rw_w = nullptr;
  float* const rw_td = nullptr;
#include "iqlhip_bwd_body.inc"
}
template <bool FULL, bool MULTI>
__global__ __launch_bounds__(256) void iql_bwd_rw_kernel(const float* q_heads, const float* q_xb, const float* q_h1, const float* q_h0,
                                                         const float* q_params, unsigned q_dims, unsigned q_ldB, unsigned q_mbc,
                                                         unsigned q_rts, StepParams p, const float* rw_w, float* rw_td) {
  constexpr bool BF16 = false;
  constexpr bool KPF = false;
  constexpr bool RW = true;
#include "iqlhip_bwd_body.inc"
}

#define IMG_W0_OFF 65536
#define IMG_STRIDE (65536 + 256 * 128)
__device__ __forceinline__ unsigned img_w1_off(int unit, int k) {
  return (unsigned)((((unit >> 6) * 4 + ((unit >> 4) & 3)) * 8 + (k >> 5)) * 512 + ((unit & 15) + 16 * ((k >> 3) & 3)) * 8 + (k & 7));
}
__device__ __forceinline__ unsigned img_w0_off(int unit, int k, int nkb) {
  return (unsigned)(IMG_W0_OFF + (((unit >> 6) * 4 + ((unit >> 4) & 3)) * nkb + (k >> 5)) * 512 + ((unit & 15) + 16 * ((k >> 3) & 3)) * 8 + (k & 7));
}
__device__ __forceinline__ void img_store4(__bf16* img, long long e, long long w1, long long w0, int k_in, const f32x4 v) {
  if (e >= w1 && e < w1 + 65536) {
    const int idx = (int)(e - w1);
    bf16x4 r;
#pragma unroll
    for (int i = 0; i < 4; ++i) r[i] = (__bf16)v[i];
    *(bf16x4*)(img + img_w1_off(idx >> 8, idx & 255)) = r;
  } else if (e >= w0 && e < w0 + 256 * k_in) {
    const int nkb = (k_in + 31) >> 5;
    const float inv_k = __builtin_amdgcn_rcpf((float)k_in);
#pragma unroll
    for (int i = 0; i < 4; ++i) {
      const int idx = (int)(e - w0) + i;
      int unit = (int)((float)idx * inv_k);
      int k = idx - unit * k_in;
      if (k < 0) { unit -= 1; k += k_in; }
      if (k >= k_in) { unit += 1; k -= k_in; }
      img[img_w0_off(unit, k, nkb)] = (__bf16)v[i];
    }
  }
}

struct UpdParams {
  iqlhip_layout L;
  iqlhip_step_scalars sc;
  float tau, one_minus_tau;
  float* params;
  float* target;
  float* m;
  float* v;
  const float* slab_a;
  const float* slab_b;
  long long slab_b_off[4];
  const float* flat_grads;
  const float* peer_flat[IQLHIP_MAX_WORLD];
  int n_peer;
  int peer_direct;
  const float* peer_slab_b[IQLHIP_MAX_WORLD];
  const float* peer_loss[IQLHIP_MAX_WORLD];
  float* loss_parts;
  float* losses;
  float* losses_mirror;
  float* loss_ring;
  int ring_slot;
  int n_chunk, n_rt;
  int n_loss;
  const float* slab_x;
  int n_x;
  int batch_rows;
  const iqlhip_step_scalars* sched;
  int sched_idx;
  const unsigned long long* ring_hdr;
  unsigned long long* adv_hdr;
  int adv_k, adv_rows;
  unsigned long long* done_flag;
// ... 241 lines not shown
  const int t = threadIdx.x;
  const unsigned long long v = (x.hdr ? x.hdr[HDR_XSTEP] : x.xstep) + (unsigned long long)k + 1ull;
  if (t < x.world && t != x.rank) {
    __builtin_amdgcn_fence(__ATOMIC_RELEASE, "");
    wait_vm0();
    __hip_atomic_store(x.peer_flags[t] + 16 * x.rank, v, __ATOMIC_RELAXED, __HIP_MEMORY_SCOPE_SYSTEM);
    const unsigned long long* mine = x.peer_flags[x.rank] + 16 * t;
    if (__hip_atomic_load(x.status, __ATOMIC_RELAXED, __HIP_MEMORY_SCOPE_AGENT) == 0ull) {
      const unsigned long long t0 = wall_clock64();
      unsigned long long polls = 0;
      while (__hip_atomic_load(mine, __ATOMIC_RELAXED, __HIP_MEMORY_SCOPE_SYSTEM) < v) {
        __builtin_amdgcn_s_sleep(4);
        if (((++polls) & 63ull) == 0ull && wall_clock64() - t0 > x.timeout_ticks) {
          __hip_atomic_store(x.status, v, __ATOMIC_RELAXED, __HIP_MEMORY_SCOPE_AGENT);
          break;
        }
      }
    }
  }
}

template <bool SYS, bool LB = false>
__global__ __launch_bounds__(256) void iql_grad_flatten_kernel(UpdParams u, float* out) {
  const long long e = ((long long)blockIdx.x * 256 + threadIdx.x) * 4;
  if (e < u.L.n_params) {
    const int net = net_of(u.L, e);
    const f32x4 gv = slab_grad<LB>(u, e, net);
    if (SYS) store16_sys(out + e, gv);
    else *(f32x4*)(out + e) = gv;
  }
  if (blockIdx.x == 0 && threadIdx.x == 0) {
    float s[4];
    loss_words(u, s);
    const float ib = u.sc.inv_batch;
    const f32x4 tail = (f32x4){s[0] * ib, (s[1] * ib + s[2] * ib) * 0.5f, s[3] * ib, 0.f};
    if (SYS) store16_sys(out + u.L.n_params, tail);
    else *(f32x4*)(out + u.L.n_params) = tail;
  }
}

#define UPD_EARLY_G 1u
template <bool FROM_TABLE, bool PEER, bool LB = false>
__global__ __launch_bounds__(256) void iql_update_kernel(float* q_p, float* q_m, float* q_v, const float* q_slab_a, unsigned q_s0,
                                                         unsigned q_s1, unsigned q_s2, unsigned q_s3, unsigned q_end,
                                                         unsigned q_flags, UpdParams u) {
  constexpr int step = 0;
  constexpr bool CLIP = false;
  const float* const q_clip = nullptr;
#include "iqlhip_upd_body.inc"
}
template <bool FROM_TABLE>
__global__ __launch_bounds__(256) void iql_update_clip_kernel(float* q_p, float* q_m, float* q_v, const float* q_slab_a, unsigned q_s0,
                                                              unsigned q_s1, unsigned q_s2, unsigned q_s3, unsigned q_end,
                                                              unsigned q_flags, const float* q_clip, UpdParams u) {
  constexpr int step = 0;
  constexpr bool PEER = false, LB = false, CLIP = true;
#include "iqlhip_upd_body.inc"
}

struct GroupRec {
  StepParams p;
  const float* q_heads; const float* q_xb; const float* q_h1; const float* q_h0; const float* q_params;
  unsigned q_dims, q_ldB, q_mbc, q_rts;
  UpdParams u;
  float* u_p; float* u_m; float* u_v; const float* u_slab_a;
  unsigned u_s0, u_s1, u_s2, u_s3, u_end, u_flags;
  const float* rows;
  long long ld, size;
  unsigned long long seed, offset;
  float* xb;
  int B;
  int n_steps;
  const float* rows_on;
  long long size_on;
  int n_off;
};

template <bool BF16, bool W0DMA, bool MULTI>
__global__ __launch_bounds__(256) __attribute__((amdgpu_waves_per_eu(2))) void iql_fwd_group_kernel(const GroupRec* __restrict__ recs) {
  constexpr bool ONE = false;
  constexpr bool ROW_EXIT = true;
  constexpr bool MIXED_IDLE = false;
  const StepParams& p = recs[blockIdx.y].p;
#include "iqlhip_fwd_body.inc"
}

template <bool BF16, bool FULL>
__global__ __launch_bounds__(256) void iql_bwd_group_kernel(const GroupRec* __restrict__ recs) {
  constexpr bool MULTI = false;
  constexpr bool KPF = false;
  constexpr bool RW = false;
  const float* const rw_w = nullptr;
  float* const rw_td = nullptr;
  const GroupRec& r = recs[blockIdx.y];
  const float* q_heads = r.q_heads; const float* q_xb = r.q_xb; const float* q_h1 = r.q_h1; const float* q_h0 = r.q_h0;
  const float* q_params = r.q_params;
  const unsigned q_dims = r.q_dims, q_ldB = r.q_ldB, q_mbc = r.q_mbc, q_rts = r.q_rts;
  const StepParams& p = r.p;
#include "iqlhip_bwd_body.inc"
}

__global__ __launch_bounds__(256) void iql_update_group_kernel(const GroupRec* __restrict__ recs, int step) {
  constexpr bool FROM_TABLE = true, PEER = false, LB = false;
  const GroupRec& r = recs[blockIdx.y];
  float* q_p = r.u_p; float* q_m = r.u_m; float* q_v = r.u_v; const float* q_slab_a = r.u_slab_a;
  const unsigned q_s0 = r.u_s0, q_s1 = r.u_s1, q_s2 = r.u_s2, q_s3 = r.u_s3, q_end = r.u_end, q_flags = r.u_flags;
  const UpdParams& u = r.u;
  step = min(max(step, 0), r.n_steps - 1);
  constexpr bool CLIP = false;
  const float* const q_clip = nullptr;
#include "iqlhip_upd_body.inc"
}

__global__ __launch_bounds__(256) void iql_gather_group_kernel(const GroupRec* __restrict__ recs, int step) {
  const GroupRec& r = recs[blockIdx.y];
  const int s = min(max(step, 0), r.n_steps - 1);
  gather_rows_drawn(r.rows, r.ld, r.xb, r.B, r.seed, r.offset, (unsigned long long)s * (unsigned long long)r.B,
                    (unsigned long long)r.size, (int)blockIdx.x * 256 + (int)threadIdx.x, (int)gridDim.x * 256);
}

struct GroupDropRec {
  unsigned* bits;
  int n_rows;
  int max_batch;
  unsigned thresh;
  int active;
  unsigned long long seed, step0;
};
__device__ __forceinline__ void group_drop_words(const GroupDropRec& d, unsigned long long step, int first, int stride) {
  const int per = d.n_rows * 8;
  for (int v = first; v < 2 * per; v += stride) {
    const int w = (v < per) ? v : d.max_batch * 8 + (v - per);
    dropmask_words(d.bits, w + 1, d.thresh, d.seed, step, w, w + 1);
  }
}

__global__ __launch_bounds__(256) void iql_dropmask_group_kernel(const GroupDropRec* __restrict__ drops) {
  const GroupDropRec& d = drops[blockIdx.y];
  group_drop_words(d, d.step0, (int)blockIdx.x * 256 + (int)threadIdx.x, (int)gridDim.x * 256);
}

__global__ __launch_bounds__(256) void iql_gather_drop_group_kernel(const GroupRec* __restrict__ recs,
                                                                    const GroupDropRec* __restrict__ drops, int step) {
  const GroupRec& r = recs[blockIdx.y];
  const int s = min(max(step, 0), r.n_steps - 1);
  gather_rows_drawn(r.rows, r.ld, r.xb, r.B, r.seed, r.offset, (unsigned long long)s * (unsigned long long)r.B,
                    (unsigned long long)r.size, (int)blockIdx.x * 256 + (int)threadIdx.x, (int)gridDim.x * 256);
  const GroupDropRec& d = drops[blockIdx.y];
  if (d.active)
    group_drop_words(d, d.step0 + (unsigned long long)s, ((int)gridDim.x - 1 - (int)blockIdx.x) * 256 + (int)threadIdx.x,
                     (int)gridDim.x * 256);
}

struct StatsArgs {
  const float* heads;
  const float* xb;
  int ld, rows, rd_off;
  float beta, discount, exp_adv_max;
  float* gparts;
  int n_part;
  float* last;
  float* ring;
  int ring_slot, ring_cap;
  const unsigned long long* ring_hdr;
};

// ... 538 lines not shown

__global__ __launch_bounds__(256) void iql_online_gather2_kernel(float* rows, const float* rows_off, long long ld,
                                                                 long long pointer, const float* row_host,
                                                                 const long long* idx_host, float* xb, int n_off, int n);

struct GroupOnlineRec {
  float* rows;
  const float* row_pin;
  const long long* idx_pin;
  float* xb;
  const float* act_pin;
  float* xb_act;
  long long ld, pointer;
  int n, S;
  const float* rows_off;
  int n_off;
};
struct GroupActRec {
  const float* heads;
  const float* log_std;
  float* out;
  float max_action, ls_min, ls_max;
  unsigned long long seed, call;
};

__device__ __forceinline__ void online_gather_member(const GroupOnlineRec& g) {
  __shared__ long long s_idx[260];
  float* rows = g.rows;
  const float* row_host = g.row_pin;
  const long long ld = g.ld, pointer = g.pointer;
  const int n = g.n;
  const int q = (int)(ld >> 2);
  const int e0 = (int)blockIdx.x * 256;
  const int r_first = e0 / q;
  const int r_last = min((e0 + 255) / q, n - 1);
  if ((int)threadIdx.x <= r_last - r_first) s_idx[threadIdx.x] = g.idx_pin[r_first + threadIdx.x];
  if (blockIdx.x == 0) {
    for (int c4 = (int)threadIdx.x; c4 < q; c4 += 256)
      *(f32x4*)(rows + pointer * ld + 4 * c4) = *(const f32x4*)(row_host + 4 * c4);
    if (g.act_pin)
      for (int c = (int)threadIdx.x; c < (int)ld; c += 256) g.xb_act[c] = (c < g.S) ? g.act_pin[c] : 0.f;
  }
  __syncthreads();
  const int e = e0 + (int)threadIdx.x;
  if (e < n * q) {
    const int r = e / q, c4 = e - r * q;
    const long long i = s_idx[r - r_first];
    const float* src = (i == pointer) ? row_host : rows + i * ld;
    *(f32x4*)(g.xb + (long long)r * ld + 4 * c4) = *(const f32x4*)(src + 4 * c4);
  }
}
__global__ __launch_bounds__(256) void iql_online_gather_group_kernel(const GroupOnlineRec* __restrict__ recs) {
  online_gather_member(recs[blockIdx.y]);
}
__global__ __launch_bounds__(256) void iql_online_gather_drop_group_kernel(const GroupOnlineRec* __restrict__ recs,
                                                                           const ActDropRec* __restrict__ drops) {
  online_gather_member(recs[blockIdx.y]);
  const ActDropRec& d = drops[blockIdx.y];
  if (d.active)
    act_drop_words(d, ((int)gridDim.x - 1 - (int)blockIdx.x) * 256 + (int)threadIdx.x, (int)gridDim.x * 256);
}

__global__ __launch_bounds__(256) void iql_online_gather2_group_kernel(const GroupOnlineRec* __restrict__ recs);
__global__ __launch_bounds__(256) void iql_online_gather2_drop_group_kernel(const GroupOnlineRec* __restrict__ recs,
                                                                            const ActDropRec* __restrict__ drops);
__global__ __launch_bounds__(256) void iql_gather2_group_kernel(const GroupRec* __restrict__ recs, int step);
__global__ __launch_bounds__(256) void iql_gather2_drop_group_kernel(const GroupRec* __restrict__ recs,
                                                                     const GroupDropRec* __restrict__ drops, int step);

struct GroupWtRec {
  WTab wt;
};
__global__ __launch_bounds__(256) void iql_gather_weighted_group_kernel(const GroupRec* __restrict__ recs,
                                                                        const GroupWtRec* __restrict__ wts, int step);
__global__ __launch_bounds__(256) void iql_gather_weighted_drop_group_kernel(const GroupRec* __restrict__ recs,
                                                                             const GroupWtRec* __restrict__ wts,
                                                                             const GroupDropRec* __restrict__ drops, int step);

template <bool BF16, bool W0DMA>
__global__ __launch_bounds__(256) __attribute__((amdgpu_waves_per_eu(2))) void iql_act_fwd_group_kernel(const StepParams* __restrict__ ps) {
  constexpr bool MULTI = false, ONE = true, ROW_EXIT = false;
  constexpr bool MIXED_IDLE = false;
  const StepParams& p = ps[blockIdx.y];
#include "iqlhip_fwd_body.inc"
}

__global__ __launch_bounds__(256) void iql_actor_finish_group_kernel(const GroupActRec* __restrict__ recs, int n_req, int A,
                                                                     unsigned long long* done_flag,
                                                                     unsigned long long done_val) {
  for (int e = (int)threadIdx.x; e < n_req * A; e += 256) {
    const int j = e / A, d = e - j * A;
    const GroupActRec& r = recs[j];
    actor_finish_elem(r.heads, d, A, r.max_action, r.log_std, r.ls_min, r.ls_max, nullptr, 0, r.seed, r.call, r.out, A);
  }
  __threadfence_system();
  __syncthreads();
  if (threadIdx.x == 0) __hip_atomic_store(done_flag, done_val, __ATOMIC_RELEASE, __HIP_MEMORY_SCOPE_SYSTEM);
}

__global__ void iql_group_done_kernel(unsigned long long* done_flag, unsigned long long done_val) {
  if (threadIdx.x == 0) __hip_atomic_store(done_flag, done_val, __ATOMIC_RELEASE, __HIP_MEMORY_SCOPE_SYSTEM);
}

struct GroupPackRec {
  float* xb;
  const float* s;
  long long ld_s;
  int ld, S, n;
};
struct GroupActRowsRec {
  const float* heads;
  const float* log_std;
  float* out;
  long long ld_out;
  int n, A;
  float max_action, ls_min, ls_max;
  unsigned long long seed, call;
};

__global__ __launch_bounds__(256) void iql_pack_states_group_kernel(const GroupPackRec* __restrict__ recs) {
  const GroupPackRec& r = recs[blockIdx.y];
  pack_states(r.xb, r.ld, r.S, r.n, r.s, r.ld_s);
}
__global__ __launch_bounds__(256) void iql_pack_states_drop_group_kernel(const GroupPackRec* __restrict__ recs,
                                                                         const ActDropRec* __restrict__ drops) {
  const GroupPackRec& r = recs[blockIdx.y];
  pack_states(r.xb, r.ld, r.S, r.n, r.s, r.ld_s);
  const ActDropRec& d = drops[blockIdx.y];
  if (d.active)
    act_drop_words(d, ((int)gridDim.x - 1 - (int)blockIdx.x) * 256 + (int)threadIdx.x, (int)gridDim.x * 256);
}

__global__ __launch_bounds__(256) void iql_actor_finish_rows_group_kernel(const GroupActRowsRec* __restrict__ recs) {
  const GroupActRowsRec& r = recs[blockIdx.y];
  const int e = blockIdx.x * blockDim.x + threadIdx.x;
  if (e < r.n * r.A)
    actor_finish_elem(r.heads, e, r.A, r.max_action, r.log_std, r.ls_min, r.ls_max, nullptr, 0, r.seed, r.call, r.out, r.ld_out);
}

template <bool BF16, bool W0DMA, bool MULTI>
__global__ __launch_bounds__(256) __attribute__((amdgpu_waves_per_eu(2))) void iql_fwd_mixed_kernel(StepParams p) {
  constexpr bool ONE = false, ROW_EXIT = false, MIXED_IDLE = true;
#include "iqlhip_fwd_body.inc"
}
```

jsrl-corl_amd/csrc/iqlhip_prio_kernels.h:

```cpp
#pragma once

__device__ __forceinline__ float td_priority(float e1, float e2, float eps, float alpha) {
  return __builtin_amdgcn_exp2f(alpha * __builtin_amdgcn_logf(fmaxf(fabsf(e1), fabsf(e2)) + eps));
}

struct PrioArgs {
  const float* words;
  float alpha, eps;
};

struct WtTd {
  const float* __restrict__ td;
  float alpha, eps;
  __device__ __forceinline__ float operator()(unsigned j) const {
    const f32x2 e = *(const f32x2*)(td + 2u * j);
    const bool finite = ((__float_as_uint(e[0]) & 0x7F800000u) != 0x7F800000u) && ((__float_as_uint(e[1]) & 0x7F800000u) != 0x7F800000u);
    return finite ? td_priority(e[0], e[1], eps, alpha) : __builtin_nanf("");
  }
};
__device__ __forceinline__ bool prio_source(const float* td, const PrioArgs& a, WtTd* out) {
  float alpha = a.alpha, eps = a.eps;
  if (a.words) {
    if (__float_as_uint(a.words[2]) == 0u) return false;
    alpha = a.words[0];
// ... 4 lines not shown
}

__global__ __launch_bounds__(256) void iql_wt_update_stamp_td_kernel(const long long* __restrict__ idx, const float* __restrict__ td,
                                                                     unsigned m, long long bound, WUpd t, PrioArgs a) {
  WtTd w;
  if (prio_source(td, a, &w)) wt_update_stamp(idx, w, m, bound, t);
}
__global__ __launch_bounds__(256) void iql_wt_update_delta_td_kernel(const long long* __restrict__ idx, const float* __restrict__ td,
                                                                     unsigned m, long long bound, WUpd t,
                                                                     unsigned long long* __restrict__ delta, PrioArgs a) {
  WtTd w;
  if (prio_source(td, a, &w)) wt_update_delta(idx, w, m, bound, t, delta);
}
__global__ __launch_bounds__(256) void iql_wt_update_apply_td_kernel(const long long* __restrict__ idx, const float* __restrict__ td,
                                                                     unsigned m, long long bound, WUpd t,
                                                                     const unsigned long long* __restrict__ delta, PrioArgs a) {
  WtTd w;
  if (prio_source(td, a, &w)) wt_update_apply(idx, w, m, bound, t, delta);
}

__device__ __forceinline__ void gather_rows_drawn_weighted_qi(const float* rows, long long ld, float* xb, float* qf, long long* ix,
                                                              int n, const WTab& wt, unsigned long long seed,
                                                              unsigned long long ctr0, unsigned long long j0, int wave, int n_waves) {
  const int q = (int)(ld >> 2);
  const int lane = (int)(threadIdx.x & 63);
  for (int r0 = wave; r0 < n; r0 += 2 * n_waves) {
    const int r1 = r0 + n_waves;
    const bool two = r1 < n;
    const unsigned long long j[2] = {j0 + (unsigned long long)r0, j0 + (unsigned long long)(two ? r1 : r0)};
    long long i[2];
    draw_index_weighted<2>(wt, seed, ctr0, j, i);
    if (lane == 0) {
      qf[r0] = (float)wt_leaf(wt, (unsigned)i[0]);
      ix[r0] = i[0];
      if (two) {
        qf[r1] = (float)wt_leaf(wt, (unsigned)i[1]);
        ix[r1] = i[1];
      }
    }
    for (int c4 = lane; c4 < q; c4 += 64) {
      const f32x4 a = *(const f32x4*)(rows + i[0] * ld + 4 * c4);
      f32x4 b = a;
      if (two) b = *(const f32x4*)(rows + i[1] * ld + 4 * c4);
      *(f32x4*)(xb + (long long)r0 * ld + 4 * c4) = a;
      if (two) *(f32x4*)(xb + (long long)r1 * ld + 4 * c4) = b;
    }
  }
}
__device__ __forceinline__ void idle_gather_weighted_qi(const IdleWork& w, unsigned long long seed, unsigned long long ctr0,
                                                        unsigned long long j0, int blk, int nblk) {
  const WTab wt = w.wt;
  const int wave = __builtin_amdgcn_readfirstlane(blk * 4 + (int)(threadIdx.x >> 6));
  gather_rows_drawn_weighted_qi(w.rows, w.ld, w.xb_dst, w.q_dst, w.idx_dst, w.n, wt, seed, ctr0, j0, wave, nblk * 4);
}

__global__ __launch_bounds__(256) void iql_call_setup_prio_kernel(unsigned long long* hdr, ChunkHdr h,
                                                                  iqlhip_step_scalars* sched_call,
                                                                  const iqlhip_step_scalars* sched_src, int n_steps,
                                                                  const float* rows, long long ld, float* xb, int B,
                                                                  unsigned* drop_dst, int drop_words, unsigned drop_thresh,
                                                                  unsigned* arrivals, unsigned long long* ack,
                                                                  unsigned long long ack_val, WTab wt, float* q_dst,
                                                                  float* beta_dev, float beta, long long* idx_dst,
                                                                  float* prio_words, float alpha, float eps, unsigned live) {
  call_setup_head(hdr, h, sched_call, sched_src, n_steps, arrivals, ack, ack_val);
  if (blockIdx.x == 0 && threadIdx.x == 0) {
    *beta_dev = beta;
    prio_words[0] = alpha;
    prio_words[1] = eps;
    prio_words[2] = __uint_as_float(live);
  }
  if (B > 0)
    gather_rows_drawn_weighted_qi(rows, ld, xb, q_dst, idx_dst, B, wt, h.w[HDR_SEED], h.w[HDR_OFFSET], h.w[HDR_POS],
                                  __builtin_amdgcn_readfirstlane((int)(blockIdx.x * 4u + (threadIdx.x >> 6))), (int)gridDim.x * 4);
  if (drop_dst)
    dropmask_words(drop_dst, drop_words, drop_thresh, h.w[HDR_DROP_SEED], h.w[HDR_DROP_STEP],
                   ((int)gridDim.x - 1 - (int)blockIdx.x) * 256 + (int)threadIdx.x, (int)gridDim.x * 256);
}

template <bool W0DMA, bool MULTI>
__global__ __launch_bounds__(256) __attribute__((amdgpu_waves_per_eu(2))) void iql_fwd_prio_kernel(StepParams p) {
  constexpr bool BF16 = false, ONE = false, ROW_EXIT = false;
  constexpr int MIXED_IDLE = 4;
#include "iqlhip_fwd_body.inc"
}
```

jsrl-corl_amd/csrc/iqlhip_weighted_kernels.h:

```cpp
#pragma once

#define WT_MAX_LEVELS 4
#define WT_SCAN_ITEMS 16
#define WT_SCAN_TILE (256 * WT_SCAN_ITEMS)


__global__ __launch_bounds__(256) void iql_wt_validate_kernel(const float* __restrict__ w, long long n, unsigned* out) {
  unsigned mx = 0u, bad = 0u;
  for (long long i = (long long)blockIdx.x * 256 + threadIdx.x; i < n; i += (long long)gridDim.x * 256) {
    const unsigned b = __float_as_uint(w[i]);
    if ((b & 0x7F800000u) == 0x7F800000u) bad |= 1u;
    else if ((b >> 31) && (b << 1)) bad |= 2u;
    else mx = max(mx, b & 0x7FFFFFFFu);
  }
#pragma unroll
  for (int o = 32; o > 0; o >>= 1) {
    mx = max(mx, (unsigned)__shfl_xor((int)mx, o));
    bad |= (unsigned)__shfl_xor((int)bad, o);
  }
  if ((threadIdx.x & 63) == 0) {
    if (mx) atomicMax(out, mx);
    if (bad) atomicOr(out + 1, bad);
  }
}
// ... 269 lines not shown
#pragma unroll
      for (int u = 0; u < U; ++u) {
        if (size[l] <= 64u) {
          const unsigned long long total = __shfl(sep[u], (int)width[u] - 1);
          t[u] = __umul64hi(r[u], total);
        }
        const unsigned child = min((unsigned)__popcll(__ballot(lane < width[u] && sep[u] <= t[u])), width[u] - 1u);
        node[u] = 64u * node[u] + child;
        if (wt.local) {
          const unsigned long long before = __shfl(sep[u], (int)max(child, 1u) - 1);
          t[u] -= child ? before : 0ull;
        }
      }
    }
  }
#pragma unroll
  for (int u = 0; u < U; ++u) out[u] = (long long)node[u];
}

__global__ __launch_bounds__(256) void iql_draw_indices_weighted_kernel(long long* idx, long long n_idx, WTab wt,
                                                                        unsigned long long seed, unsigned long long offset) {
  const long long wave = __builtin_amdgcn_readfirstlane((int)(blockIdx.x * 4u + (threadIdx.x >> 6)));
  const long long n_waves = (long long)gridDim.x * 4;
  for (long long j0 = wave; j0 < n_idx; j0 += 2 * n_waves) {
    const long long j1 = j0 + n_waves;
    const unsigned long long j[2] = {(unsigned long long)j0, (unsigned long long)(j1 < n_idx ? j1 : j0)};
    long long i[2];
    draw_index_weighted<2>(wt, seed, offset, j, i);
    if ((threadIdx.x & 63) == 0) {
      idx[j0] = i[0];
      if (j1 < n_idx) idx[j1] = i[1];
    }
  }
}

__device__ __forceinline__ void gather_rows_drawn_weighted(const float* rows, long long ld, float* xb, int n, const WTab& wt,
                                                           unsigned long long seed, unsigned long long ctr0,
                                                           unsigned long long j0, int wave, int n_waves) {
  const int q = (int)(ld >> 2);
  const int lane = (int)(threadIdx.x & 63);
  for (int r0 = wave; r0 < n; r0 += 2 * n_waves) {
    const int r1 = r0 + n_waves;
    const bool two = r1 < n;
    const unsigned long long j[2] = {j0 + (unsigned long long)r0, j0 + (unsigned long long)(two ? r1 : r0)};
    long long i[2];
    draw_index_weighted<2>(wt, seed, ctr0, j, i);
    for (int c4 = lane; c4 < q; c4 += 64) {
      const f32x4 a = *(const f32x4*)(rows + i[0] * ld + 4 * c4);
      f32x4 b = a;
      if (two) b = *(const f32x4*)(rows + i[1] * ld + 4 * c4);
      *(f32x4*)(xb + (long long)r0 * ld + 4 * c4) = a;
      if (two) *(f32x4*)(xb + (long long)r1 * ld + 4 * c4) = b;
    }
  }
}

__device__ __forceinline__ void idle_gather_weighted(const IdleWork& w, unsigned long long seed, unsigned long long ctr0,
                                                     unsigned long long j0, int blk, int nblk) {
  const WTab wt = w.wt;
  const int wave = __builtin_amdgcn_readfirstlane(blk * 4 + (int)(threadIdx.x >> 6));
  gather_rows_drawn_weighted(w.rows, w.ld, w.xb_dst, w.n, wt, seed, ctr0, j0, wave, nblk * 4);
}

__global__ __launch_bounds__(256) void iql_call_setup_weighted_kernel(unsigned long long* hdr, ChunkHdr h,
                                                                      iqlhip_step_scalars* sched_call,
                                                                      const iqlhip_step_scalars* sched_src, int n_steps,
                                                                      const float* rows, long long ld, float* xb, int B,
                                                                      unsigned* drop_dst, int drop_words, unsigned drop_thresh,
                                                                      unsigned* arrivals, unsigned long long* ack,
                                                                      unsigned long long ack_val, WTab wt) {
  call_setup_head(hdr, h, sched_call, sched_src, n_steps, arrivals, ack, ack_val);
  if (B > 0)
    gather_rows_drawn_weighted(rows, ld, xb, B, wt, h.w[HDR_SEED], h.w[HDR_OFFSET], h.w[HDR_POS],
                               __builtin_amdgcn_readfirstlane((int)(blockIdx.x * 4u + (threadIdx.x >> 6))), (int)gridDim.x * 4);
  if (drop_dst)
    dropmask_words(drop_dst, drop_words, drop_thresh, h.w[HDR_DROP_SEED], h.w[HDR_DROP_STEP],
                   ((int)gridDim.x - 1 - (int)blockIdx.x) * 256 + (int)threadIdx.x, (int)gridDim.x * 256);
}

template <bool BF16, bool W0DMA, bool MULTI>
__global__ __launch_bounds__(256) __attribute__((amdgpu_waves_per_eu(2))) void iql_fwd_weighted_kernel(StepParams p) {
  constexpr bool ONE = false, ROW_EXIT = false;
  constexpr int MIXED_IDLE = 2;
#include "iqlhip_fwd_body.inc"
}

__device__ __forceinline__ void group_gather_weighted(const GroupRec& r, const GroupWtRec& w, int s) {
  const unsigned long long j0 = (unsigned long long)s * (unsigned long long)r.B;
  if (w.wt.tab) {
    const WTab wt = w.wt;
    const int wave = __builtin_amdgcn_readfirstlane((int)(blockIdx.x * 4u + (threadIdx.x >> 6)));
    gather_rows_drawn_weighted(r.rows, r.ld, r.xb, r.B, wt, r.seed, r.offset, j0, wave, (int)gridDim.x * 4);
  } else {
    gather_rows_drawn(r.rows, r.ld, r.xb, r.B, r.seed, r.offset, j0, (unsigned long long)r.size,
                      (int)blockIdx.x * 256 + (int)threadIdx.x, (int)gridDim.x * 256);
  }
}

__global__ __launch_bounds__(256) void iql_gather_weighted_group_kernel(const GroupRec* __restrict__ recs,
                                                                        const GroupWtRec* __restrict__ wts, int step) {
  const GroupRec& r = recs[blockIdx.y];
  const int s = min(max(step, 0), r.n_steps - 1);
  group_gather_weighted(r, wts[blockIdx.y], s);
}

__global__ __launch_bounds__(256) void iql_gather_weighted_drop_group_kernel(const GroupRec* __restrict__ recs,
                                                                             const GroupWtRec* __restrict__ wts,
                                                                             const GroupDropRec* __restrict__ drops, int step) {
  const GroupRec& r = recs[blockIdx.y];
  const int s = min(max(step, 0), r.n_steps - 1);
  group_gather_weighted(r, wts[blockIdx.y], s);
  const GroupDropRec& d = drops[blockIdx.y];
  if (d.active)
    group_drop_words(d, d.step0 + (unsigned long long)s, ((int)gridDim.x - 1 - (int)blockIdx.x) * 256 + (int)threadIdx.x,
                     (int)gridDim.x * 256);
}
```

jsrl-corl_amd/iqlhip_binding.py:

```python
from __future__ import annotations

import ctypes as C
import os
from typing import Optional

_HERE = os.path.dirname(os.path.abspath(__file__))
LIB_PATH = os.environ.get("IQLHIP_LIB", os.path.join(_HERE, "libiqlhip.so"))

IQLHIP_HIDDEN = 256
IQLHIP_ACT_ROWS = 4096
IQLHIP_MAX_WORLD = 8
IQLHIP_GRAPH_STEPS = 64
IQLHIP_N_STATS = 16
STAT_NAMES = ("v_mean", "next_v_mean", "q1_mean", "q2_mean", "target_q_mean", "td_target_mean", "q_gap_mean",
              "adv_mean", "adv_min", "adv_max", "adv_pos_frac", "exp_adv_mean", "exp_adv_clamped_frac",
              "grad_norm_vf", "grad_norm_qf", "grad_norm_actor")
IQLHIP_N_SCORE = 8
SCORE_NAMES = ("v", "next_v", "q1", "q2", "target_q", "adv", "exp_adv", "bc")
SPREAD_NAMES = tuple("mean_" + name for name in SCORE_NAMES) + tuple("std_" + name for name in SCORE_NAMES)
IQLHIP_MAX_GROUP = 16
IQLHIP_GROUP_ACT_WAIT = 1
IQLHIP_GROUP_DROPOUT = 1
IQLHIP_GROUP_MAX_STEPS = 1024
IQLHIP_GROUP_TS_CONTINUE = 1
# ... 95 lines not shown
    ("iqlhip_train_steps_prepare", C.c_int, [C.c_void_p, C.c_void_p, C.c_int64, C.c_int32, C.c_float, C.c_void_p]),
    ("iqlhip_comm_unique_id", C.c_int, [C.c_void_p]),
    ("iqlhip_allreduce_init", C.c_int, [C.c_void_p, C.c_void_p, C.c_int, C.c_int]),
    ("iqlhip_p2p_export", C.c_int, [C.c_void_p, C.c_void_p, C.c_int, C.c_int]),
    ("iqlhip_p2p_attach", C.c_int, [C.c_void_p, C.c_void_p, C.c_int]),
    ("iqlhip_xch_select", C.c_int, [C.c_void_p, C.c_int]),
    ("iqlhip_xch_status", C.c_int, [C.c_void_p, C.POINTER(C.c_int64), C.c_void_p]),
    ("iqlhip_xch_clear_status", C.c_int, [C.c_void_p, C.c_void_p]),
    ("iqlhip_xch_shutdown", C.c_int, [C.c_void_p]),
    ("iqlhip_read_losses", C.c_int, [C.c_void_p, C.POINTER(C.c_float), C.c_void_p]),
    ("iqlhip_read_loss_ring", C.c_int, [C.c_void_p, C.POINTER(C.c_float), C.c_int32, C.c_void_p]),
    ("iqlhip_row_stride", C.c_int64, [C.c_int32, C.c_int32]),
    ("iqlhip_rows_write", C.c_int, [C.c_void_p, C.c_int64, C.c_int32, C.c_int32, C.c_int64, C.c_int64,
                                    C.c_void_p, C.c_void_p, C.c_void_p, C.c_void_p, C.c_void_p, C.c_void_p]),
    ("iqlhip_rows_fill_synth", C.c_int, [C.c_void_p, C.c_int64, C.c_int32, C.c_int32, C.c_int64, C.c_int64, C.c_uint64,
                                         C.c_float, C.c_int32, C.c_void_p]),
    ("iqlhip_rows_gather", C.c_int, [C.c_void_p, C.c_int64, C.c_int64, C.c_int32, C.c_int32, C.c_void_p, C.c_int64,
                                     C.c_void_p, C.c_void_p, C.c_void_p, C.c_void_p, C.c_void_p, C.c_void_p]),
    ("iqlhip_actor_forward", C.c_int, [C.c_void_p, C.c_void_p, C.c_int64, C.c_int32, C.c_void_p, C.c_int64, C.c_float,
                                       C.c_void_p, C.c_int64, C.c_void_p]),
    ("iqlhip_rows_gather_packed", C.c_int, [C.c_void_p, C.c_int64, C.c_int64, C.c_void_p, C.c_int64, C.c_void_p, C.c_void_p]),
    ("iqlhip_actor_sample", C.c_int, [C.c_void_p, C.c_void_p, C.c_int64, C.c_int32, C.c_uint64, C.c_float, C.c_void_p,
                                      C.c_int64, C.c_void_p]),
    ("iqlhip_stream_synchronize", C.c_int, [C.c_void_p]),
    ("iqlhip_rows_gather_packed_h", C.c_int, [C.c_void_p, C.c_int64, C.c_int64, C.c_void_p, C.c_void_p, C.c_int64, C.c_void_p,
                                              C.c_void_p]),
    ("iqlhip_rows_sample_packed", C.c_int, [C.c_void_p, C.c_int64, C.c_int64, C.c_void_p, C.c_int64, C.c_void_p, C.c_void_p]),
    ("iqlhip_cols_mean_std", C.c_int, [C.c_void_p, C.c_int64, C.c_int32, C.c_int64, C.c_float, C.c_void_p, C.c_void_p,
                                       C.c_void_p]),
    ("iqlhip_rows_normalize", C.c_int, [C.c_void_p, C.c_int64, C.c_int32, C.c_int32, C.c_int64, C.c_int64, C.c_void_p,
                                        C.c_void_p, C.c_void_p]),
    ("iqlhip_rows_return_range", C.c_int, [C.c_void_p, C.c_int64, C.c_int32, C.c_int32, C.c_int64, C.c_int64, C.c_int32,
                                           C.POINTER(C.c_double), C.POINTER(C.c_int64), C.c_void_p]),
    ("iqlhip_rows_reward_scale", C.c_int, [C.c_void_p, C.c_int64, C.c_int32, C.c_int32, C.c_int64, C.c_int64, C.c_float,
                                           C.c_float, C.c_void_p]),
    ("iqlhip_rows_reward_shift", C.c_int, [C.c_void_p, C.c_int64, C.c_int32, C.c_int32, C.c_int64, C.c_int64, C.c_float,
                                           C.c_void_p]),
    ("iqlhip_rows_episode_returns", C.c_int, [C.c_void_p, C.c_int64, C.c_int32, C.c_int32, C.c_int64, C.c_int64, C.c_int64,
                                              C.c_double, C.c_double, C.c_int32, C.POINTER(C.c_double), C.c_void_p,
                                              C.c_void_p, C.c_void_p, C.c_void_p, C.POINTER(C.c_int64), C.c_void_p]),
    ("iqlhip_draw_indices", C.c_int, [C.c_void_p, C.c_int64, C.c_int64, C.c_uint64, C.c_uint64, C.c_void_p]),
    ("iqlhip_weights_build", C.c_int, [C.c_void_p, C.c_int64, C.c_void_p, C.POINTER(C.c_void_p)]),
    ("iqlhip_weights_free", C.c_int, [C.c_void_p]),
    ("iqlhip_weights_info", C.c_int, [C.c_void_p, C.POINTER(C.c_int64), C.POINTER(C.c_uint64), C.POINTER(C.c_int32),
                                      C.POINTER(C.c_uint64), C.c_void_p]),
    ("iqlhip_weights_build_updatable", C.c_int, [C.c_void_p, C.c_int64, C.c_int64, C.c_float, C.c_void_p,
                                                 C.POINTER(C.c_void_p)]),
    ("iqlhip_weights_update", C.c_int, [C.c_void_p, C.c_void_p, C.c_void_p, C.c_int64, C.c_int64, C.c_void_p]),
    ("iqlhip_weights_clear_flags", C.c_int, [C.c_void_p, C.c_void_p]),
    ("iqlhip_weights_state", C.c_int, [C.c_void_p, C.POINTER(C.c_uint64), C.POINTER(C.c_uint32), C.POINTER(C.c_uint64),
                                       C.c_void_p]),
    ("iqlhip_draw_indices_weighted", C.c_int, [C.c_void_p, C.c_int64, C.c_void_p, C.c_uint64, C.c_uint64, C.c_void_p]),
    ("iqlhip_train_steps_weighted", C.c_int, [C.c_void_p, C.c_void_p, C.c_int64, C.c_int64, C.c_int32, C.c_void_p,
                                              C.c_int32, C.c_uint64, C.c_uint64, C.c_int32, C.c_void_p, C.c_void_p]),
    ("iqlhip_train_steps_weighted_is", C.c_int, [C.c_void_p, C.c_void_p, C.c_int64, C.c_int64, C.c_int32, C.c_void_p,
                                                 C.c_int32, C.c_uint64, C.c_uint64, C.c_int32, C.c_void_p, C.c_void_p,
                                                 C.c_float]),
    ("iqlhip_train_steps_weighted_is_prepare", C.c_int, [C.c_void_p, C.c_void_p, C.c_int64, C.c_int32, C.c_float,
                                                         C.c_void_p, C.c_void_p]),
    ("iqlhip_train_steps_weighted_prepare", C.c_int, [C.c_void_p, C.c_void_p, C.c_int64, C.c_int32, C.c_float, C.c_void_p,
                                                      C.c_void_p]),
    ("iqlhip_weights_update_td", C.c_int, [C.c_void_p, C.c_void_p, C.c_void_p, C.c_int64, C.c_int64, C.c_float, C.c_float,
                                           C.c_void_p]),
    ("iqlhip_train_steps_prioritized", C.c_int, [C.c_void_p, C.c_void_p, C.c_int64, C.c_int64, C.c_int32, C.c_void_p,
                                                 C.c_int32, C.c_uint64, C.c_uint64, C.c_int32, C.c_void_p, C.c_void_p,
                                                 C.c_float, C.c_float, C.c_float]),
    ("iqlhip_train_steps_prioritized_prepare", C.c_int, [C.c_void_p, C.c_void_p, C.c_int64, C.c_int32, C.c_float,
                                                         C.c_void_p, C.c_void_p]),
    ("iqlhip_weights_build_tracking", C.c_int, [C.c_void_p, C.c_int64, C.c_int64, C.c_float, C.c_float, C.c_void_p,
                                                C.POINTER(C.c_void_p)]),
    ("iqlhip_weights_max", C.c_int, [C.c_void_p, C.POINTER(C.c_uint64), C.POINTER(C.c_float)]),
    ("iqlhip_weights_insert_max", C.c_int, [C.c_void_p, C.c_int64, C.c_int64, C.c_void_p]),
    ("iqlhip_online_step_prioritized", C.c_int, [C.c_void_p, C.c_void_p, C.c_int64, C.c_int64, C.c_int64, C.c_void_p,
                                                 C.c_int32, C.POINTER(StepScalars), C.POINTER(C.c_float), C.c_void_p, C.c_float,
                                                 C.c_uint64, C.c_void_p, C.c_void_p, C.c_void_p, C.c_uint64, C.c_uint64,
                                                 C.c_float, C.c_float, C.c_float]),
    ("iqlhip_online_prioritized_batch", C.c_int, [C.c_void_p, C.c_int32, C.c_void_p, C.c_void_p, C.c_void_p]),
    ("iqlhip_debug_read", C.c_int, [C.c_void_p, C.c_char_p, C.POINTER(C.c_float), C.c_int64,
                                    C.POINTER(C.c_int64), C.c_void_p]),
    ("iqlhip_debug_time_kernel", C.c_int, [C.c_void_p, C.POINTER(Batch), C.c_int, C.c_int, C.POINTER(C.c_float),
                                           C.c_void_p]),
    ("iqlhip_debug_drain_spin", C.c_int, [C.c_void_p, C.c_void_p, C.POINTER(C.c_double)]),
    ("iqlhip_debug_live_buffers", C.c_int64, []),
    ("iqlhip_group_create", C.c_int, [C.POINTER(C.c_void_p), C.c_int, C.POINTER(C.c_void_p)]),
    ("iqlhip_group_create_flags", C.c_int, [C.POINTER(C.c_void_p), C.c_int, C.c_int32, C.POINTER(C.c_void_p)]),
    ("iqlhip_group_destroy", C.c_int, [C.c_void_p]),
    ("iqlhip_group_step", C.c_int, [C.c_void_p, C.POINTER(Batch), C.POINTER(StepScalars), C.POINTER(C.c_float), C.c_void_p]),
    ("iqlhip_group_train_steps", C.c_int, [C.c_void_p, C.POINTER(C.c_void_p), C.c_int64, C.POINTER(C.c_int64), C.c_int32,
                                           C.POINTER(C.c_void_p), C.c_int32, C.POINTER(C.c_uint64), C.POINTER(C.c_uint64),
                                           C.c_int32, C.c_void_p]),
    ("iqlhip_group_step_mixed", C.c_int, [C.c_void_p, C.POINTER(Batch), C.POINTER(StepScalars), C.POINTER(C.c_float),
                                          C.c_void_p]),
    ("iqlhip_group_train_steps_mixed", C.c_int, [C.c_void_p, C.POINTER(C.c_void_p), C.c_int64, C.POINTER(C.c_int64),
                                                 C.POINTER(C.c_int32), C.POINTER(C.c_void_p), C.c_int32,
                                                 C.POINTER(C.c_uint64), C.POINTER(C.c_uint64), C.c_int32, C.c_void_p]),
    ("iqlhip_group_online_step_mixed", C.c_int, [C.c_void_p, C.POINTER(C.c_void_p), C.c_int64, C.POINTER(C.c_int64),
                                                 C.POINTER(C.c_int64), C.c_void_p, C.c_void_p, C.POINTER(C.c_int32),
                                                 C.POINTER(StepScalars), C.POINTER(C.c_float), C.c_void_p, C.c_void_p,
                                                 C.c_void_p, C.c_void_p, C.c_void_p, C.c_void_p]),
    ("iqlhip_group_read_losses", C.c_int, [C.c_void_p, C.POINTER(C.c_float), C.c_int32, C.c_void_p]),
    ("iqlhip_group_online_step", C.c_int, [C.c_void_p, C.POINTER(C.c_void_p), C.c_int64, C.POINTER(C.c_int64),
                                           C.POINTER(C.c_int64), C.c_void_p, C.c_void_p, C.c_int32,
                                           C.POINTER(StepScalars), C.POINTER(C.c_float), C.c_void_p, C.c_void_p,
                                           C.c_void_p, C.c_void_p, C.c_void_p, C.c_void_p]),
    ("iqlhip_group_online_step_replay2", C.c_int, [C.c_void_p, C.POINTER(C.c_void_p), C.c_int64, C.POINTER(C.c_int64),
                                                   C.POINTER(C.c_int64), C.c_void_p, C.c_void_p, C.POINTER(C.c_int32),
                                                   C.POINTER(StepScalars), C.POINTER(C.c_float), C.c_void_p, C.c_void_p,
                                                   C.c_void_p, C.c_void_p, C.c_void_p, C.c_void_p, C.POINTER(C.c_void_p),
                                                   C.POINTER(C.c_int64), C.POINTER(C.c_int32)]),
    ("iqlhip_group_train_steps_replay2", C.c_int, [C.c_void_p, C.POINTER(C.c_void_p), C.POINTER(C.c_int64),
                                                   C.POINTER(C.c_void_p), C.POINTER(C.c_int64), C.c_int64,
                                                   C.POINTER(C.c_int32), C.POINTER(C.c_int32), C.POINTER(C.c_void_p),
                                                   C.c_int32, C.POINTER(C.c_uint64), C.POINTER(C.c_uint64), C.c_void_p]),
    ("iqlhip_group_train_steps_weighted", C.c_int, [C.c_void_p, C.POINTER(C.c_void_p), C.c_int64, C.POINTER(C.c_int64),
                                                    C.POINTER(C.c_int32), C.POINTER(C.c_void_p), C.c_int32,
                                                    C.POINTER(C.c_uint64), C.POINTER(C.c_uint64), C.c_int32, C.c_void_p,
                                                    C.POINTER(C.c_void_p)]),
    ("iqlhip_group_step_rw", C.c_int, [C.c_void_p, C.POINTER(Batch), C.POINTER(StepScalars), C.POINTER(C.c_void_p),
                                       C.POINTER(C.c_void_p), C.POINTER(C.c_float), C.c_void_p]),
    ("iqlhip_group_train_steps_weighted_is", C.c_int, [C.c_void_p, C.POINTER(C.c_void_p), C.c_int64, C.POINTER(C.c_int64),
                                                       C.POINTER(C.c_int32), C.POINTER(C.c_void_p), C.c_int32,
                                                       C.POINTER(C.c_uint64), C.POINTER(C.c_uint64), C.c_int32, C.c_void_p,
                                                       C.POINTER(C.c_void_p), C.POINTER(C.c_float)]),
    ("iqlhip_group_train_steps_prioritized", C.c_int, [C.c_void_p, C.POINTER(C.c_void_p), C.c_int64, C.POINTER(C.c_int64),
                                                       C.POINTER(C.c_int32), C.POINTER(C.c_void_p), C.c_int32,
                                                       C.POINTER(C.c_uint64), C.POINTER(C.c_uint64), C.c_int32, C.c_void_p,
                                                       C.POINTER(C.c_void_p), C.POINTER(C.c_float), C.POINTER(C.c_float),
                                                       C.POINTER(C.c_float)]),
    ("iqlhip_group_actor_forward", C.c_int, [C.c_void_p, C.POINTER(C.c_void_p), C.c_int64, C.POINTER(C.c_int32),
                                             C.POINTER(C.c_uint64), C.POINTER(C.c_float), C.POINTER(C.c_void_p),
                                             C.c_int64, C.c_int32, C.c_void_p]),
    ("iqlhip_set_step_stats", C.c_int, [C.c_void_p, C.c_int]),
    ("iqlhip_read_step_stats", C.c_int, [C.c_void_p, C.POINTER(C.c_float), C.c_void_p]),
    ("iqlhip_read_stats_ring", C.c_int, [C.c_void_p, C.POINTER(C.c_float), C.c_int32, C.c_void_p]),
    ("iqlhip_group_read_step_stats", C.c_int, [C.c_void_p, C.POINTER(C.c_float), C.c_int32, C.c_void_p]),
    ("iqlhip_set_grad_clip", C.c_int, [C.c_void_p, C.POINTER(C.c_float)]),
    ("iqlhip_get_grad_clip", C.c_int, [C.c_void_p, C.POINTER(C.c_float)]),
    ("iqlhip_read_grad_clip", C.c_int, [C.c_void_p, C.POINTER(C.c_float), C.c_void_p]),
    ("iqlhip_score_rows", C.c_int, [C.c_void_p, C.c_void_p, C.c_int64, C.c_int64, C.c_int64, C.c_int64, C.c_void_p,
                                    C.c_void_p, C.c_int32, C.POINTER(C.c_float), C.c_void_p]),
    ("iqlhip_pack_rows", C.c_int, [C.c_void_p, C.POINTER(Batch), C.c_void_p, C.c_void_p]),
    ("iqlhip_group_score_rows", C.c_int, [C.c_void_p, C.POINTER(C.c_void_p), C.c_int64, C.POINTER(C.c_int64), C.c_int64,
                                          C.c_int64, C.POINTER(C.c_void_p), C.POINTER(C.c_void_p), C.c_void_p, C.c_int32,
                                          C.POINTER(C.c_float), C.c_void_p]),
    ("iqlhip_jsrl_create", C.c_int, [C.POINTER(C.c_void_p), C.POINTER(C.c_void_p), C.POINTER(C.c_void_p), C.c_int,
                                     C.POINTER(C.c_void_p)]),
    ("iqlhip_jsrl_destroy", C.c_int, [C.c_void_p]),
    ("iqlhip_jsrl_act", C.c_int, [C.c_void_p, C.POINTER(C.c_void_p), C.c_int64, C.POINTER(C.c_int32), C.POINTER(C.c_void_p),
                                  C.POINTER(C.c_float), C.POINTER(C.c_uint64), C.POINTER(C.c_float), C.POINTER(C.c_float),
                                  C.POINTER(C.c_void_p), C.c_int64, C.POINTER(C.c_void_p), C.POINTER(C.c_void_p), C.c_int32,
                                  C.c_void_p]),
    ("iqlhip_jsrl_online_step", C.c_int, [C.c_void_p, C.c_void_p, C.c_int64, C.c_int64, C.c_int64, C.c_void_p, C.c_void_p,
                                          C.c_int32, C.POINTER(StepScalars), C.POINTER(C.c_float), C.c_void_p, C.c_int8,
                                          C.c_float, C.c_uint64, C.c_float, C.c_float, C.c_void_p, C.POINTER(C.c_int32),
                                          C.POINTER(C.c_float), C.c_void_p]),
    ("iqlhip_set_timing", C.c_int, [C.c_void_p, C.c_int]),
    ("iqlhip_get_timing", C.c_int, [C.c_void_p, C.POINTER(C.c_float)]),
    ("iqlhip_var_layout", C.c_int, [C.c_int32, C.POINTER(NetLayout), C.POINTER(C.c_int64)]),
    ("iqlhip_var_create", C.c_int, [C.c_int32, C.c_int32, C.c_int, C.POINTER(C.c_void_p)]),
    ("iqlhip_var_destroy", C.c_int, [C.c_void_p]),
    ("iqlhip_var_bind", C.c_int, [C.c_void_p, C.c_void_p, C.c_void_p, C.c_void_p]),
    ("iqlhip_var_step", C.c_int, [C.c_void_p, C.c_void_p, C.c_int32, C.c_int32, C.POINTER(VarScalars), C.c_void_p]),
    ("iqlhip_var_values", C.c_int, [C.c_void_p, C.c_void_p, C.c_int32, C.c_int32, C.c_void_p, C.c_void_p]),
    ("iqlhip_var_forward_backward", C.c_int, [C.c_void_p, C.c_void_p, C.c_int32, C.c_int32, C.c_int32, C.c_void_p,
                                              C.c_void_p]),
    ("iqlhip_var_read_loss", C.c_int, [C.c_void_p, C.POINTER(C.c_float), C.POINTER(C.c_float), C.c_int32, C.c_void_p]),
# ... 86 lines not shown
```

Before: 52130 steps/s.

## Add early-issue forward kernel variant computing weight pointers from arena layout

Adds a specialized forward kernel that receives a few scalars (param bases, dims, ld/rows packed) as direct kernel arguments and derives per-network weight pointers from the fixed arena layout, so global loads of inputs and the first W1 fragments can be issued before reading the large StepParams struct. It checks at create time and per launch that the layout matches the assumed packing, and falls back to the original kernel otherwise. The aim is to hide kernel-argument and pointer-chasing latency at the start of each forward block, at the cost of more code paths, an extra kernel variant and a per-launch validation check on the host.

```diff
diff --git a/include/iqlhip.h b/include/iqlhip.h
--- a/include/iqlhip.h
+++ b/include/iqlhip.h
@@ -347,6 +347,7 @@
                              void* stream);
 int iqlhip_debug_drain_spin(iqlhip_ctx* ctx, void* stream, double* spin_us);
 int64_t iqlhip_debug_live_buffers(void);
+int64_t iqlhip_debug_fwd_early_launches(const iqlhip_ctx* ctx);
 int iqlhip_set_timing(iqlhip_ctx* ctx, int enabled);
 int iqlhip_get_timing(iqlhip_ctx* ctx, float out_us[4]);
 
diff --git a/jsrl-corl_amd/csrc/iqlhip.hip b/jsrl-corl_amd/csrc/iqlhip.hip
--- a/jsrl-corl_amd/csrc/iqlhip.hip
+++ b/jsrl-corl_amd/csrc/iqlhip.hip
@@ -211,6 +211,9 @@
   int bwd_donate_pct = -1;
   int bwd_spb_force = -1;
   int fwd_spb_force = -1;
+  bool fwd_early = true;
+  bool fwd_early_layout = false;
+  mutable std::atomic<int64_t> fwd_early_launches{0};
   float* pi_t = nullptr;
   __bf16* dh1g = nullptr;
   float* slab_x = nullptr;
@@ -329,6 +332,7 @@
 extern "C" int iqlhip_destroy(iqlhip_ctx* c);
 extern "C" int iqlhip_xch_shutdown(iqlhip_ctx* c);
 
+static bool fwd_early_layout_ok(const iqlhip_ctx* c);
 static int create_impl(iqlhip_ctx* c, const iqlhip_dims* dims, const iqlhip_hyper* hyper, int device) {
   c->dims = *dims;
   c->hyper = *hyper;
@@ -396,6 +400,7 @@
   if (const char* ov = getenv("IQLHIP_BWD_DONATE_PCT")) c->bwd_donate_pct = std::max(0, std::min(100, atoi(ov)));
   if (const char* ov = getenv("IQLHIP_BWD_SPB_L2")) c->bwd_spb_force = std::max(0, std::min(2, atoi(ov)));
   if (const char* ov = getenv("IQLHIP_FWD_SPB_L2")) c->fwd_spb_force = std::max(0, std::min(2, atoi(ov)));
+  if (const char* ov = getenv("IQLHIP_FWD_EARLY")) c->fwd_early = atoi(ov) != 0;
   if (const char* ov = getenv("IQLHIP_LB")) c->lb_enabled = atoi(ov) != 0;
   if (const char* ov = getenv("IQLHIP_LB_NBB")) c->lb_nbb_force = std::max(2, atoi(ov));
   if (const char* ov = getenv("IQLHIP_LB_CSPLIT")) c->lb_csplit = atoi(ov) != 0;
@@ -415,11 +420,13 @@
   c->lds_bwd = std::max(lds_a, lds_b);
   c->lds_bwd_lb = (size_t)(3 * 32 * H0B_LD + 32 * LB_DYLD) * 2 + 32 * 4 + (size_t)(2 * 4 * 32 + 16) * 4;
   int rc = set_max_lds(3, c->lds_fwd_solo, [](unsigned m) { return fwd_kernel(m & 1, m & 2, m & 4); });
+  if (!rc) rc = set_max_lds(0, c->lds_fwd_solo, [](unsigned) { return &iql_fwd_kernel_early; });
   if (!rc) rc = set_max_lds(2, c->lds_fwd_solo, [](unsigned m) { return fwd_one_kernel(m & 1, m & 2); });
   if (!rc) rc = set_max_lds(3, c->lds_bwd, [](unsigned m) { return bwd_kernel(m & 1, m & 2, m & 4); });
   if (!rc) rc = set_max_lds(1, c->lds_bwd_lb, [](unsigned m) { return bwd_rows_kernel(m & 1); });
   if (!rc) rc = set_max_lds(2, c->lds_bwd, [](unsigned m) { return bwd_rw_kernel(m & 1, m & 2); });
   c->fwd_lds_set[(int)ChunkKind::Plain] = !rc;
+  c->fwd_early_layout = fwd_early_layout_ok(c);
   return rc;
 }
 
@@ -778,9 +785,53 @@
 static size_t fwd_lds(const iqlhip_ctx* c, int n_blocks) { return (n_blocks <= c->n_cus) ? c->lds_fwd_solo : c->lds_fwd; }
 
 static const void* fwd_kernel_of(ChunkKind kind, bool bf, bool dma, bool multi);
+extern "C" int64_t iqlhip_debug_fwd_early_launches(const iqlhip_ctx* ctx) {
+  return ctx ? ctx->fwd_early_launches.load(std::memory_order_relaxed) : -1;
+}
+static bool fwd_early_layout_ok(const iqlhip_ctx* c) {
+  const iqlhip_layout& L = c->L;
+  const int S = c->dims.state_dim, A = c->dims.action_dim, kq = S + A;
+  if (kq > FWD_EARLY_MAX_K || kq > c->w0_lds_k || c->w0_lds_k > W0_LDS_MAX_K) return false;
+  if (RT_ROWS * c->row_ld / 4 > 3 * 256 || S > 255 || A > 63 || c->row_ld > 1023) return false;
+  long long begin = 0;
+  for (int n = 0; n < 4; ++n) {
+    const iqlhip_net_layout& nl = L.net[n];
+    const long long k0 = nl.k_in, d = nl.d_out;
+    if (k0 != ((n == IQLHIP_NET_Q1 || n == IQLHIP_NET_Q2) ? kq : S) || d != (n == IQLHIP_NET_PI ? A : 1)) return false;
+    if (nl.seg_begin != begin || nl.w1 != begin || nl.w0 != begin + 65536 || nl.b0 != nl.w0 + 256 * k0 || nl.b1 != nl.b0 + 256 ||
+        nl.w2 != nl.b1 + 256 || nl.b2 != nl.w2 + 256 * d)
+      return false;
+    const long long seg_n = (65536 + 256 * k0 + 512 + 256 * d + ((d + 3) & ~3LL) + 63) & ~63LL;
+    if (n != IQLHIP_NET_PI && nl.seg_end != begin + seg_n) return false;
+    begin = nl.seg_end;
+  }
+  return true;
+}
+static bool fwd_early_ok(const iqlhip_ctx* c, const StepParams& p, ChunkKind kind, bool bf, bool dma, bool multi) {
+  if (!c->fwd_early || !c->fwd_early_layout || kind != ChunkKind::Plain || bf || dma || multi || p.only_inst >= 0) return false;
+  if (p.S != c->dims.state_dim || p.A != c->dims.action_dim || p.ld != (int)c->row_ld || p.rows >= (1 << 22)) return false;
+  const float* tb = c->target - c->L.target_src;
+  const int netof[7] = {IQLHIP_NET_V, IQLHIP_NET_V, IQLHIP_NET_Q1, IQLHIP_NET_Q2, IQLHIP_NET_Q1, IQLHIP_NET_Q2, IQLHIP_NET_PI};
+  for (int i = 0; i < 7; ++i)
+    if (p.inst[i].w1 != ((i == 2 || i == 3) ? tb : c->params) + c->L.net[netof[i]].w1) return false;
+  return true;
+}
 static void launch_fwd_grid(const iqlhip_ctx* c, const StepParams& p, int nb, hipStream_t st, ChunkKind kind = ChunkKind::Plain) {
   const bool dma = c->w0_lds_k > W0_LDS_MAX_K;
   const bool bf = c->precision == 1, multi = (p.spb_l2 & 3) > 0;
+  if (fwd_early_ok(c, p, kind, bf, dma, multi)) {
+    const float* q_params = c->params;
+    const float* q_target = c->target - c->L.target_src;
+    const float* q_xb = p.xb;
+    const unsigned* q_drop = p.drop_bits;
+    unsigned q_dims = (unsigned)p.S | ((unsigned)p.A << 8) | ((unsigned)p.policy << 14);
+    unsigned q_ldB = (unsigned)p.ld | ((unsigned)p.rows << 10);
+    unsigned q_mb = (unsigned)p.sc.max_batch;
+    void* args[] = {&q_params, &q_target, &q_xb, &q_drop, &q_dims, &q_ldB, &q_mb, const_cast<StepParams*>(&p)};
+    (void)hipLaunchKernel((const void*)&iql_fwd_kernel_early, dim3(nb), dim3(256), args, fwd_lds(c, nb), st);
+    c->fwd_early_launches.fetch_add(1, std::memory_order_relaxed);
+    return;
+  }
   const void* kernel = (p.only_inst >= 0) ? (const void*)fwd_one_kernel(bf, dma) : fwd_kernel_of(kind, bf, dma, multi);
   void* args[] = {const_cast<StepParams*>(&p)};
   (void)hipLaunchKernel(kernel, dim3(nb), dim3(256), args, fwd_lds(c, nb), st);
diff --git a/jsrl-corl_amd/csrc/iqlhip_fwd_body.inc b/jsrl-corl_amd/csrc/iqlhip_fwd_body.inc
--- a/jsrl-corl_amd/csrc/iqlhip_fwd_body.inc
+++ b/jsrl-corl_amd/csrc/iqlhip_fwd_body.inc
@@ -30,25 +30,33 @@
   const int tid = threadIdx.x, lane = tid & 63, wave = tid >> 6;
   const int l15 = lane & 15, g = lane >> 4;
 
-  const NetPtrs np = p.inst[inst];
-  const int xoff = p.xoff[inst];
-  const int slot = p.slot[inst];
+  const int e_net = (inst < 2) ? IQLHIP_NET_V : ((inst == 6) ? IQLHIP_NET_PI : IQLHIP_NET_Q1 + (inst & 1));
+  const ArenaOff e_ao = arena_off(EARLY ? e_net : 0, (int)(q_dims & 255u), (int)((q_dims >> 8) & 63u),
+                                  (int)((q_dims >> 14) & 1u) == IQLHIP_POLICY_GAUSSIAN);
+  const float* const e_base = (inst == 2 || inst == 3) ? q_target : q_params;
+  const NetPtrs np = EARLY ? NetPtrs{e_base + e_ao.w0, e_base + e_ao.b0, e_base + (e_ao.w0 - 65536u), e_base + e_ao.b1,
+                                     e_base + e_ao.w2, e_base + e_ao.b2, e_ao.k0, e_ao.d}
+                           : p.inst[inst];
+  int xoff = EARLY ? 0 : p.xoff[inst];
+  int slot = EARLY ? -1 : p.slot[inst];
   const int k0 = np.k0;
   const int k0p = (k0 + 3) & ~3;
   const int D = np.d;
-  const int ld = p.ld;
-  const int B = p.rows;
-  const int w0k = p.w0_lds_k;
-  const float* xb = p.xb;
-  float* h0g = p.sc.h0;
-  float* h1g = p.sc.h1;
-  float* headsg = p.sc.heads;
-  const int MB = p.sc.max_batch;
-  const int Aact = p.A;
-  PIN_P(np.w0); PIN_P(np.b0); PIN_P(np.w1); PIN_P(np.b1); PIN_P(np.w2); PIN_P(np.b2);
-  PIN_S(k0); PIN_S(D); PIN_S(xoff); PIN_S(slot); PIN_S(ld); PIN_S(B); PIN_S(MB); PIN_S(Aact);
-  PIN_P(xb); PIN_P(h0g); PIN_P(h1g); PIN_P(headsg); PIN_S(w0k);
-  const bool w0_lds = W0DMA ? (k0 <= w0k) : (k0 <= min(w0k, W0_LDS_MAX_K));
+  const int ld = EARLY ? (int)(q_ldB & 1023u) : p.ld;
+  const int B = EARLY ? (int)(q_ldB >> 10) : p.rows;
+  const int w0k = EARLY ? FWD_EARLY_MAX_K : p.w0_lds_k;
+  const float* xb = EARLY ? q_xb : p.xb;
+  float* h0g = EARLY ? nullptr : p.sc.h0;
+  float* h1g = EARLY ? nullptr : p.sc.h1;
+  float* headsg = EARLY ? nullptr : p.sc.heads;
+  const int MB = EARLY ? (int)q_mb : p.sc.max_batch;
+  const int Aact = EARLY ? (int)((q_dims >> 8) & 63u) : p.A;
+  if constexpr (!EARLY) {
+    PIN_P(np.w0); PIN_P(np.b0); PIN_P(np.w1); PIN_P(np.b1); PIN_P(np.w2); PIN_P(np.b2);
+    PIN_S(k0); PIN_S(D); PIN_S(xoff); PIN_S(slot); PIN_S(ld); PIN_S(B); PIN_S(MB); PIN_S(Aact);
+    PIN_P(xb); PIN_P(h0g); PIN_P(h1g); PIN_P(headsg); PIN_S(w0k);
+  }
+  const bool w0_lds = EARLY ? true : (W0DMA ? (k0 <= w0k) : (k0 <= min(w0k, W0_LDS_MAX_K)));
   const bool w0_dma = W0DMA && w0_lds && (k0 > W0_LDS_MAX_K);
 
   extern __shared__ __attribute__((aligned(16))) float smem[];
@@ -65,7 +73,13 @@
   const int n_x = RT_ROWS * ld / 4;
   const int x_last = B * ld / 4 - 1;
   f32x4 xr[XR_MAX_F4];
-  xr_load(xr, xb, row0 * ld / 4, n_x, x_last);
+  if constexpr (EARLY) {
+#pragma unroll
+    for (int q = 0; q < XR_MAX_F4; ++q) xr[q] = (f32x4){0.f, 0.f, 0.f, 0.f};
+    xr_issue<0, 3>(xr, xb, row0 * ld / 4, n_x, x_last);
+  } else {
+    xr_load(xr, xb, row0 * ld / 4, n_x, x_last);
+  }
   f32x4 w2pre[2];
 #pragma unroll
   for (int q = 0; q < 2; ++q) {
@@ -77,9 +91,16 @@
 #pragma unroll
   for (int ct = 0; ct < 4; ++ct) bias0[ct] = *(const f32x4*)(np.b0 + (unsigned)(wave * 64 + ct * 16 + 4 * g));
   f32x4 bias1 = *(const f32x4*)(np.b1 + (unsigned)(ns * 64 + wave * 16 + 4 * g));
-  const bool drop = (inst == 6) && (p.drop_bits != nullptr);
+  const bool drop = (inst == 6) && ((EARLY ? q_drop : p.drop_bits) != nullptr);
   unsigned mk0 = 0xFFFFFFFFu, mk1 = 0xFFFFFFFFu;
-  if (drop) {
+  if constexpr (EARLY) {
+    const int mrow = min(row0 + (tid >> 3), B - 1);
+    const unsigned* const dsrc = drop ? q_drop : (const unsigned*)q_xb;
+    const unsigned l0w = *(dsrc + (unsigned)(drop ? mrow * 8 + (tid & 7) : 0));
+    const unsigned l1w = *(dsrc + (unsigned)(drop ? (MB + mrow) * 8 + (tid & 7) : 0));
+    mk0 = l0w;
+    mk1 = l1w;
+  } else if (drop) {
     const int mrow = min(row0 + (tid >> 3), B - 1);
     mk0 = p.drop_bits[mrow * 8 + (tid & 7)];
     mk1 = p.drop_bits[(MB + mrow) * 8 + (tid & 7)];
@@ -93,7 +114,7 @@
   } else if (w0_lds) {
 #pragma unroll
     for (int j = 0; j < 8; ++j) w0v[j] = *(const f32x4*)(np.w0 + 4u * (unsigned)min(tid + 256 * j, n_w0v - 1));
-    if (k0 > 32) {
+    if (!EARLY && k0 > 32) {
 #pragma unroll
       for (int j = 8; j < 16; ++j) w0v[j] = *(const f32x4*)(np.w0 + 4u * (unsigned)min(tid + 256 * j, n_w0v - 1));
     }
@@ -102,6 +123,21 @@
   f32x4 bw[BF16 ? 1 : 16];
   bf16x8 bwb[BF16 ? 8 : 1];
   __bf16* H0b = (__bf16*)H0s;
+#define BW_LOAD(ks_) bw[ks_] = *(const f32x4*)(np.w1 + (unsigned)(n1 * HID + 16 * (ks_) + 4 * g))
+#define BWB_AT(unit_, j_) (*(const bf16x8*)((const __bf16*)np.w1 + (unsigned)((unit_) * HID + 32 * (j_) + 8 * g)))
+  if constexpr (EARLY) {
+    __builtin_amdgcn_sched_barrier(0);
+#pragma unroll
+    for (int ks = 0; ks < FWD_EARLY_W1; ++ks) BW_LOAD(ks);
+    __builtin_amdgcn_sched_barrier(0);
+    xoff = p.xoff[inst];
+    slot = p.slot[inst];
+    h0g = p.sc.h0;
+    h1g = p.sc.h1;
+    headsg = p.sc.heads;
+    PIN_S(xoff); PIN_S(slot); PIN_P(h0g); PIN_P(h1g); PIN_P(headsg); PIN_S(p.drop_scale);
+    __builtin_amdgcn_sched_barrier(0);
+  }
 
   xr_store(xr, Xr, n_x);
   const int Dp = (D + 15) & ~15;
@@ -111,6 +147,11 @@
     if (e < Dp * 16) *(f32x4*)(W2s + (e >> 4) * W2_LD + 4 * (e & 15)) = (e < D * 16) ? w2pre[q] : (f32x4){0.f, 0.f, 0.f, 0.f};
   }
   if (tid < D) W2s[Dp * W2_LD + tid] = b2v;
+  if constexpr (EARLY) {
+    asm volatile("" : "+v"(mk0), "+v"(mk1));
+    mk0 = drop ? mk0 : 0xFFFFFFFFu;
+    mk1 = drop ? mk1 : 0xFFFFFFFFu;
+  }
   Mk[tid] = mk0;
   Mk[256 + tid] = mk1;
   if (w0_lds && !w0_dma) {
@@ -119,7 +160,7 @@
       const int f = tid + 256 * j;
       if (f < n_w0v) *(f32x4*)(W0s + 4 * f) = w0v[j];
     }
-    if (k0 > 32) {
+    if (!EARLY && k0 > 32) {
 #pragma unroll
       for (int j = 8; j < 16; ++j) {
         const int f = tid + 256 * j;
@@ -129,8 +170,6 @@
   }
   __syncthreads();
   const bool bw_in_l0 = !BF16 && w0_lds;
-#define BW_LOAD(ks_) bw[ks_] = *(const f32x4*)(np.w1 + (unsigned)(n1 * HID + 16 * (ks_) + 4 * g))
-#define BWB_AT(unit_, j_) (*(const bf16x8*)((const __bf16*)np.w1 + (unsigned)((unit_) * HID + 32 * (j_) + 8 * g)))
   if constexpr (BF16) {
 #pragma unroll
     for (int j = 0; j < 8; ++j) bwb[j] = BWB_AT(n1, j);
@@ -150,7 +189,7 @@
     const float* x0 = Xr + l15 * ld + xoff;
     const float* x1 = Xr + (16 + l15) * ld + xoff;
     float bcur[4], bnxt[4], acur[2], anxt[2];
-    if (w0_lds && nks <= 8) {
+    if (w0_lds && (EARLY || nks <= 8)) {
       const float* wl[4];
 #pragma unroll
       for (int ct = 0; ct < 4; ++ct) wl[ct] = W0s + (wave * 64 + ct * 16 + l15) * k0;
@@ -184,7 +223,9 @@
           }
           if (ks < 4) {
 #pragma unroll
-            for (int k2 = 4 * ks; k2 < 4 * ks + 4; ++k2) BW_LOAD(k2);
+            for (int k2 = 4 * ks; k2 < 4 * ks + 4; ++k2) {
+              if (!EARLY || k2 >= FWD_EARLY_W1) BW_LOAD(k2);
+            }
           }
         }
       }
@@ -298,6 +339,12 @@
   STAMP(p, 7);
   __syncthreads();
   STAMP(p, 2);
+#ifdef IQL_STAMPS
+  if constexpr (!MULTI) {
+    asm volatile("s_waitcnt vmcnt(0)" ::: "memory");
+    STAMP(p, 13);
+  }
+#endif
 
   for (int it = 0;; ++it) {
   const bool more = MULTI && (it + 1 < spb);
diff --git a/jsrl-corl_amd/csrc/iqlhip_isweight_kernels.h b/jsrl-corl_amd/csrc/iqlhip_isweight_kernels.h
--- a/jsrl-corl_amd/csrc/iqlhip_isweight_kernels.h
+++ b/jsrl-corl_amd/csrc/iqlhip_isweight_kernels.h
@@ -104,5 +104,6 @@
 __global__ __launch_bounds__(256) __attribute__((amdgpu_waves_per_eu(2))) void iql_fwd_weighted_is_kernel(StepParams p) {
   constexpr bool BF16 = false, ONE = false, ROW_EXIT = false;
   constexpr int MIXED_IDLE = 3;
+  FWD_NOT_EARLY();
 #include "iqlhip_fwd_body.inc"
 }
diff --git a/jsrl-corl_amd/csrc/iqlhip_kernels.h b/jsrl-corl_amd/csrc/iqlhip_kernels.h
--- a/jsrl-corl_amd/csrc/iqlhip_kernels.h
+++ b/jsrl-corl_amd/csrc/iqlhip_kernels.h
@@ -144,6 +144,14 @@
 
 #define PIN_S(x) asm volatile("" ::"s"(x))
 #define PIN_P(x) asm volatile("" ::"s"((unsigned long long)(uintptr_t)(x)))
+#define FWD_EARLY_MAX_K 32
+#define FWD_EARLY_W1 4
+static_assert(FWD_EARLY_W1 >= 0 && FWD_EARLY_W1 <= 16, "a wave has 16 W1 fragments");
+#define FWD_NOT_EARLY()                                                                                   \
+  constexpr bool EARLY = false;                                                                           \
+  constexpr const float *q_params = nullptr, *q_target = nullptr, *q_xb = nullptr;                        \
+  constexpr const unsigned* q_drop = nullptr;                                                             \
+  constexpr unsigned q_dims = 0, q_ldB = 0, q_mb = 0
 
 #define XR_MAX_F4 9
 #define XR_LD_MAX 260
@@ -331,171 +339,6 @@
                    (nblk - 1 - blk) * 256 + (int)threadIdx.x, nblk * 256);
 }
 
-__device__ __forceinline__ void l0_chunk_bf16(f32x4 (&acc)[2][4], const float (&bq)[8][4], const float (&aq)[8][2]) {
-  bf16x8 B[2];
-#pragma unroll
-  for (int r = 0; r < 2; ++r) {
-    float t8[8];
-#pragma unroll
-    for (int e = 0; e < 8; ++e) t8[e] = aq[e][r];
-    B[r] = pack8s(t8);
-  }
-#pragma unroll
-  for (int ct = 0; ct < 4; ++ct) {
-    float t8[8];
-#pragma unroll
-    for (int e = 0; e < 8; ++e) t8[e] = bq[e][ct];
-    const bf16x8 A = pack8s(t8);
-    acc[0][ct] = MFMA_BF16(A, B[0], acc[0][ct]);
-    acc[1][ct] = MFMA_BF16(A, B[1], acc[1][ct]);
-  }
-}
-
-template <bool BF16, bool W0DMA, bool MULTI, bool ONE = false>
-__global__ __launch_bounds__(256) __attribute__((amdgpu_waves_per_eu(2))) void iql_fwd_kernel(StepParams p) {
-  constexpr bool ROW_EXIT = false;
-  constexpr bool MIXED_IDLE = false;
-#include "iqlhip_fwd_body.inc"
-}
-
-struct RowIn {
-  f32x4 h[6];
-  float r, d;
-};
-
-__device__ __forceinline__ void row_issue(const StepParams& p, int row, RowIn& in) {
-  const float* hb = p.sc.heads;
-  const unsigned o = (unsigned)row * (unsigned)HEAD_LD;
-#pragma unroll
-  for (int i = 0; i < 6; ++i) in.h[i] = *(const f32x4*)(hb + (o + 4u * i));
-  const float* xb = p.xb;
-  const unsigned ox = (unsigned)row * (unsigned)p.ld + (unsigned)(2 * p.S + p.A);
-  in.r = xb[ox];
-  in.d = xb[ox + 1u];
-}
-
-__device__ __forceinline__ void row_issue_hot(const float* heads, const float* xb, int ld, int S, int A, int row, RowIn& in) {
-  const unsigned o = (unsigned)row * (unsigned)HEAD_LD;
-#pragma unroll
-  for (int i = 0; i < 6; ++i) in.h[i] = *(const f32x4*)(heads + (o + 4u * i));
-  const unsigned ox = (unsigned)row * (unsigned)ld + (unsigned)(2 * S + A);
-  in.r = xb[ox];
-  in.d = xb[ox + 1u];
-}
-
-__device__ __forceinline__ float sum4(const f32x4 v) { return ((v[0] + v[1]) + v[2]) + v[3]; }
-
-__device__ __forceinline__ float tanh_via_exp(float x) {
-  const float e = __builtin_amdgcn_exp2f(x * 2.885390081777927f);
-  return 1.f - 2.f * __builtin_amdgcn_rcpf(e + 1.f);
-}
-
-struct PiConst { float ls, ivar; };
-__device__ __forceinline__ float pi_ls_issue(const StepParams& p) {
-  const float* src = (p.policy == IQLHIP_POLICY_GAUSSIAN) ? p.log_std : p.xb;
-  return src[min((int)(threadIdx.x & 63), p.A - 1)];
-}
-__device__ __forceinline__ float pi_ls_issue_hot(const float* log_std, const float* xb, int policy, int A) {
-  const float* src = (policy == IQLHIP_POLICY_GAUSSIAN) ? log_std : xb;
-  return src[min((int)(threadIdx.x & 63), A - 1)];
-}
-__device__ __forceinline__ PiConst pi_consts_hot(const StepParams& p, int policy, int net, float lsr) {
-  PiConst c;
-  c.ls = 0.f;
-  c.ivar = 1.f;
-  if (net == IQLHIP_NET_PI && policy == IQLHIP_POLICY_GAUSSIAN) {
-    c.ls = fminf(fmaxf(lsr, p.hy.log_std_min), p.hy.log_std_max);
-    const float sig = expf(c.ls);
-    c.ivar = 1.f / (sig * sig);
-  }
-  return c;
-}
-__device__ __forceinline__ PiConst pi_consts(const StepParams& p, int net, float lsr) {
-  PiConst c;
-  c.ls = 0.f;
-  c.ivar = 1.f;
-  if (net == IQLHIP_NET_PI && p.policy == IQLHIP_POLICY_GAUSSIAN) {
-    c.ls = fminf(fmaxf(lsr, p.hy.log_std_min), p.hy.log_std_max);
-    const float sig = expf(c.ls);
-    c.ivar = 1.f / (sig * sig);
-  }
-  return c;
-}
-
-__device__ __forceinline__ void row_finish(const StepParams& p, int net, const RowIn& in, float* dyrow,
-                                           float& lossA, float& lossB) {
-  const float invB = p.inv_batch;
-  lossA = 0.f;
-  lossB = 0.f;
-  if (net == IQLHIP_NET_V) {
-    const float tq = fminf(sum4(in.h[2]), sum4(in.h[3]));
-    const float u = tq - sum4(in.h[1]);
-    const float wgt = fabsf(p.hy.iql_tau - ((u < 0.f) ? 1.f : 0.f));
-    lossA = wgt * u * u;
-    dyrow[0] = (-2.f * wgt * u) * invB;
-    return;
-  }
-  const float nv = sum4(in.h[0]);
-  const float y = in.r + ((1.f - in.d) * p.hy.discount) * nv;
-  const float e1 = sum4(in.h[4]) - y;
-  const float e2 = sum4(in.h[5]) - y;
-  lossA = e1 * e1;
-  lossB = e2 * e2;
-  dyrow[0] = ((net == IQLHIP_NET_Q1) ? e1 : e2) * invB;
-}
-__device__ __forceinline__ f32x2 row_td_errors(const StepParams& p, const RowIn& in) {
-  const float nv = sum4(in.h[0]);
-  const float y = in.r + ((1.f - in.d) * p.hy.discount) * nv;
-  return (f32x2){sum4(in.h[4]) - y, sum4(in.h[5]) - y};
-}
-
-__device__ __forceinline__ float block_sum_256(float v, float* red ) {
-#pragma unroll
-  for (int o = 32; o > 0; o >>= 1) v += __shfl_xor(v, o);
-  __syncthreads();
-  if ((threadIdx.x & 63) == 0) red[threadIdx.x >> 6] = v;
-  __syncthreads();
-  return (red[0] + red[1]) + (red[2] + red[3]);
-}
-
-template <int NK>
-__device__ __forceinline__ void dh1_mfma(f32x4 (&pre)[4][2], const float* dYs, const float* W2s, int DYA, int wave,
-                                         int g, int l15) {
-#pragma unroll
-  for (int k1 = 0; k1 < NK; ++k1) {
-    float a1[4];
-#pragma unroll
-    for (int t = 0; t < 4; ++t) a1[t] = dYs[(64 * wave + 16 * t + l15) * DYA + 4 * k1 + g];
-    const f32x2 b1 = *(const f32x2*)(W2s + (4 * k1 + g) * 32 + 2 * l15);
-#pragma unroll
-    for (int t = 0; t < 4; ++t) {
-      pre[t][0] = MFMA16(a1[t], b1[0], pre[t][0]);
-      pre[t][1] = MFMA16(a1[t], b1[1], pre[t][1]);
-    }
-  }
-}
-
-__device__ __forceinline__ void pi_items8(const f32x4 (&hv)[8], const float (&acv)[8], const float (&wv)[8], bool live,
-                                          bool gauss, float ivar, float ls, float invB, float (&dyv)[8], float (&dlv)[8],
-                                          float& lossA) {
-#pragma unroll
-  for (int cc = 0; cc < 8; ++cc) {
-    const float w = wv[cc];
-    const float mu = tanh_via_exp(sum4(hv[cc]));
-    const float diff = acv[cc] - mu;
-    const float q = diff * diff * ivar;
-    const float l_g = w * (0.5f * q + ls + 0.918938533204672742f);
-    const float l_d = w * (diff * diff);
-    const float dmu_g = (-(w * diff) * ivar) * invB;
-    const float dmu_d = (-2.f * w * diff) * invB;
-    const float dmu = gauss ? dmu_g : dmu_d;
-    lossA += live ? (gauss ? l_g : l_d) : 0.f;
-    dyv[cc] = live ? dmu * (1.f - mu * mu) : 0.f;
-    dlv[cc] = (live && gauss) ? w * (1.f - q) : 0.f;
-  }
-}
-
-#define BROW(r) (FULL ? (r) : min((r), B - 1))
 struct ArenaOff { unsigned w0, b0, b1, w2, b2, log_std; int k0, d; };
 __device__ __forceinline__ ArenaOff arena_off(int net, int S, int A, bool gauss) {
   auto seg = [&](int k, int d, bool ls) -> unsigned {
@@ -515,6 +358,180 @@
   o.log_std = o.b2 + (((unsigned)o.d + 3u) & ~3u);
   return o;
 }
+
+__device__ __forceinline__ void l0_chunk_bf16(f32x4 (&acc)[2][4], const float (&bq)[8][4], const float (&aq)[8][2]) {
+  bf16x8 B[2];
+#pragma unroll
+  for (int r = 0; r < 2; ++r) {
+    float t8[8];
+#pragma unroll
+    for (int e = 0; e < 8; ++e) t8[e] = aq[e][r];
+    B[r] = pack8s(t8);
+  }
+#pragma unroll
+  for (int ct = 0; ct < 4; ++ct) {
+    float t8[8];
+#pragma unroll
+    for (int e = 0; e < 8; ++e) t8[e] = bq[e][ct];
+    const bf16x8 A = pack8s(t8);
+    acc[0][ct] = MFMA_BF16(A, B[0], acc[0][ct]);
+    acc[1][ct] = MFMA_BF16(A, B[1], acc[1][ct]);
+  }
+}
+
+template <bool BF16, bool W0DMA, bool MULTI, bool ONE = false>
+__global__ __launch_bounds__(256) __attribute__((amdgpu_waves_per_eu(2))) void iql_fwd_kernel(StepParams p) {
+  constexpr bool ROW_EXIT = false;
+  constexpr bool MIXED_IDLE = false;
+  FWD_NOT_EARLY();
+#include "iqlhip_fwd_body.inc"
+}
+__global__ __launch_bounds__(256) __attribute__((amdgpu_waves_per_eu(2))) void iql_fwd_kernel_early(
+    const float* q_params, const float* q_target, const float* q_xb, const unsigned* q_drop, unsigned q_dims, unsigned q_ldB,
+    unsigned q_mb, StepParams p) {
+  constexpr bool BF16 = false, W0DMA = false, MULTI = false, ONE = false, ROW_EXIT = false, MIXED_IDLE = false;
+  constexpr bool EARLY = true;
+#include "iqlhip_fwd_body.inc"
+}
+
+struct RowIn {
+  f32x4 h[6];
+  float r, d;
+};
+
+__device__ __forceinline__ void row_issue(const StepParams& p, int row, RowIn& in) {
+  const float* hb = p.sc.heads;
+  const unsigned o = (unsigned)row * (unsigned)HEAD_LD;
+#pragma unroll
+  for (int i = 0; i < 6; ++i) in.h[i] = *(const f32x4*)(hb + (o + 4u * i));
+  const float* xb = p.xb;
+  const unsigned ox = (unsigned)row * (unsigned)p.ld + (unsigned)(2 * p.S + p.A);
+  in.r = xb[ox];
+  in.d = xb[ox + 1u];
+}
+
+__device__ __forceinline__ void row_issue_hot(const float* heads, const float* xb, int ld, int S, int A, int row, RowIn& in) {
+  const unsigned o = (unsigned)row * (unsigned)HEAD_LD;
+#pragma unroll
+  for (int i = 0; i < 6; ++i) in.h[i] = *(const f32x4*)(heads + (o + 4u * i));
+  const unsigned ox = (unsigned)row * (unsigned)ld + (unsigned)(2 * S + A);
+  in.r = xb[ox];
+  in.d = xb[ox + 1u];
+}
+
+__device__ __forceinline__ float sum4(const f32x4 v) { return ((v[0] + v[1]) + v[2]) + v[3]; }
+
+__device__ __forceinline__ float tanh_via_exp(float x) {
+  const float e = __builtin_amdgcn_exp2f(x * 2.885390081777927f);
+  return 1.f - 2.f * __builtin_amdgcn_rcpf(e + 1.f);
+}
+
+struct PiConst { float ls, ivar; };
+__device__ __forceinline__ float pi_ls_issue(const StepParams& p) {
+  const float* src = (p.policy == IQLHIP_POLICY_GAUSSIAN) ? p.log_std : p.xb;
+  return src[min((int)(threadIdx.x & 63), p.A - 1)];
+}
+__device__ __forceinline__ float pi_ls_issue_hot(const float* log_std, const float* xb, int policy, int A) {
+  const float* src = (policy == IQLHIP_POLICY_GAUSSIAN) ? log_std : xb;
+  return src[min((int)(threadIdx.x & 63), A - 1)];
+}
+__device__ __forceinline__ PiConst pi_consts_hot(const StepParams& p, int policy, int net, float lsr) {
+  PiConst c;
+  c.ls = 0.f;
+  c.ivar = 1.f;
+  if (net == IQLHIP_NET_PI && policy == IQLHIP_POLICY_GAUSSIAN) {
+    c.ls = fminf(fmaxf(lsr, p.hy.log_std_min), p.hy.log_std_max);
+    const float sig = expf(c.ls);
+    c.ivar = 1.f / (sig * sig);
+  }
+  return c;
+}
+__device__ __forceinline__ PiConst pi_consts(const StepParams& p, int net, float lsr) {
+  PiConst c;
+  c.ls = 0.f;
+  c.ivar = 1.f;
+  if (net == IQLHIP_NET_PI && p.policy == IQLHIP_POLICY_GAUSSIAN) {
+    c.ls = fminf(fmaxf(lsr, p.hy.log_std_min), p.hy.log_std_max);
+    const float sig = expf(c.ls);
+    c.ivar = 1.f / (sig * sig);
+  }
+  return c;
+}
+
+__device__ __forceinline__ void row_finish(const StepParams& p, int net, const RowIn& in, float* dyrow,
+                                           float& lossA, float& lossB) {
+  const float invB = p.inv_batch;
+  lossA = 0.f;
+  lossB = 0.f;
+  if (net == IQLHIP_NET_V) {
+    const float tq = fminf(sum4(in.h[2]), sum4(in.h[3]));
+    const float u = tq - sum4(in.h[1]);
+    const float wgt = fabsf(p.hy.iql_tau - ((u < 0.f) ? 1.f : 0.f));
+    lossA = wgt * u * u;
+    dyrow[0] = (-2.f * wgt * u) * invB;
+    return;
+  }
+  const float nv = sum4(in.h[0]);
+  const float y = in.r + ((1.f - in.d) * p.hy.discount) * nv;
+  const float e1 = sum4(in.h[4]) - y;
+  const float e2 = sum4(in.h[5]) - y;
+  lossA = e1 * e1;
+  lossB = e2 * e2;
+  dyrow[0] = ((net == IQLHIP_NET_Q1) ? e1 : e2) * invB;
+}
+__device__ __forceinline__ f32x2 row_td_errors(const StepParams& p, const RowIn& in) {
+  const float nv = sum4(in.h[0]);
+  const float y = in.r + ((1.f - in.d) * p.hy.discount) * nv;
+  return (f32x2){sum4(in.h[4]) - y, sum4(in.h[5]) - y};
+}
+
+__device__ __forceinline__ float block_sum_256(float v, float* red ) {
+#pragma unroll
+  for (int o = 32; o > 0; o >>= 1) v += __shfl_xor(v, o);
+  __syncthreads();
+  if ((threadIdx.x & 63) == 0) red[threadIdx.x >> 6] = v;
+  __syncthreads();
+  return (red[0] + red[1]) + (red[2] + red[3]);
+}
+
+template <int NK>
+__device__ __forceinline__ void dh1_mfma(f32x4 (&pre)[4][2], const float* dYs, const float* W2s, int DYA, int wave,
+                                         int g, int l15) {
+#pragma unroll
+  for (int k1 = 0; k1 < NK; ++k1) {
+    float a1[4];
+#pragma unroll
+    for (int t = 0; t < 4; ++t) a1[t] = dYs[(64 * wave + 16 * t + l15) * DYA + 4 * k1 + g];
+    const f32x2 b1 = *(const f32x2*)(W2s + (4 * k1 + g) * 32 + 2 * l15);
+#pragma unroll
+    for (int t = 0; t < 4; ++t) {
+      pre[t][0] = MFMA16(a1[t], b1[0], pre[t][0]);
+      pre[t][1] = MFMA16(a1[t], b1[1], pre[t][1]);
+    }
+  }
+}
+
+__device__ __forceinline__ void pi_items8(const f32x4 (&hv)[8], const float (&acv)[8], const float (&wv)[8], bool live,
+                                          bool gauss, float ivar, float ls, float invB, float (&dyv)[8], float (&dlv)[8],
+                                          float& lossA) {
+#pragma unroll
+  for (int cc = 0; cc < 8; ++cc) {
+    const float w = wv[cc];
+    const float mu = tanh_via_exp(sum4(hv[cc]));
+    const float diff = acv[cc] - mu;
+    const float q = diff * diff * ivar;
+    const float l_g = w * (0.5f * q + ls + 0.918938533204672742f);
+    const float l_d = w * (diff * diff);
+    const float dmu_g = (-(w * diff) * ivar) * invB;
+    const float dmu_d = (-2.f * w * diff) * invB;
+    const float dmu = gauss ? dmu_g : dmu_d;
+    lossA += live ? (gauss ? l_g : l_d) : 0.f;
+    dyv[cc] = live ? dmu * (1.f - mu * mu) : 0.f;
+    dlv[cc] = (live && gauss) ? w * (1.f - q) : 0.f;
+  }
+}
+
+#define BROW(r) (FULL ? (r) : min((r), B - 1))
 template <bool BF16, bool FULL, bool MULTI>
 __global__ __launch_bounds__(256) void iql_bwd_kernel(const float* q_heads, const float* q_xb, const float* q_h1, const float* q_h0,
                                                       const float* q_params, unsigned q_dims, unsigned q_ldB, unsigned q_mbc,
@@ -922,6 +939,7 @@
   constexpr bool ROW_EXIT = true;
   constexpr bool MIXED_IDLE = false;
   const StepParams& p = recs[blockIdx.y].p;
+  FWD_NOT_EARLY();
 #include "iqlhip_fwd_body.inc"
 }
 
@@ -1626,6 +1644,7 @@
   constexpr bool MULTI = false, ONE = true, ROW_EXIT = false;
   constexpr bool MIXED_IDLE = false;
   const StepParams& p = ps[blockIdx.y];
+  FWD_NOT_EARLY();
 #include "iqlhip_fwd_body.inc"
 }
 
@@ -1685,5 +1704,6 @@
 template <bool BF16, bool W0DMA, bool MULTI>
 __global__ __launch_bounds__(256) __attribute__((amdgpu_waves_per_eu(2))) void iql_fwd_mixed_kernel(StepParams p) {
   constexpr bool ONE = false, ROW_EXIT = false, MIXED_IDLE = true;
+  FWD_NOT_EARLY();
 #include "iqlhip_fwd_body.inc"
 }
diff --git a/jsrl-corl_amd/csrc/iqlhip_prio_kernels.h b/jsrl-corl_amd/csrc/iqlhip_prio_kernels.h
--- a/jsrl-corl_amd/csrc/iqlhip_prio_kernels.h
+++ b/jsrl-corl_amd/csrc/iqlhip_prio_kernels.h
@@ -110,5 +110,6 @@
 __global__ __launch_bounds__(256) __attribute__((amdgpu_waves_per_eu(2))) void iql_fwd_prio_kernel(StepParams p) {
   constexpr bool BF16 = false, ONE = false, ROW_EXIT = false;
   constexpr int MIXED_IDLE = 4;
+  FWD_NOT_EARLY();
 #include "iqlhip_fwd_body.inc"
 }
diff --git a/jsrl-corl_amd/csrc/iqlhip_weighted_kernels.h b/jsrl-corl_amd/csrc/iqlhip_weighted_kernels.h
--- a/jsrl-corl_amd/csrc/iqlhip_weighted_kernels.h
+++ b/jsrl-corl_amd/csrc/iqlhip_weighted_kernels.h
@@ -375,6 +375,7 @@
 __global__ __launch_bounds__(256) __attribute__((amdgpu_waves_per_eu(2))) void iql_fwd_weighted_kernel(StepParams p) {
   constexpr bool ONE = false, ROW_EXIT = false;
   constexpr int MIXED_IDLE = 2;
+  FWD_NOT_EARLY();
 #include "iqlhip_fwd_body.inc"
 }
 
diff --git a/jsrl-corl_amd/iqlhip_binding.py b/jsrl-corl_amd/iqlhip_binding.py
--- a/jsrl-corl_amd/iqlhip_binding.py
+++ b/jsrl-corl_amd/iqlhip_binding.py
@@ -201,6 +201,7 @@
                                            C.c_void_p]),
     ("iqlhip_debug_drain_spin", C.c_int, [C.c_void_p, C.c_void_p, C.POINTER(C.c_double)]),
     ("iqlhip_debug_live_buffers", C.c_int64, []),
+    ("iqlhip_debug_fwd_early_launches", C.c_int64, [C.c_void_p]),
     ("iqlhip_group_create", C.c_int, [C.POINTER(C.c_void_p), C.c_int, C.POINTER(C.c_void_p)]),
     ("iqlhip_group_create_flags", C.c_int, [C.POINTER(C.c_void_p), C.c_int, C.c_int32, C.POINTER(C.c_void_p)]),
     ("iqlhip_group_destroy", C.c_int, [C.c_void_p]),
```

After: 52810 steps/s (median of 6 runs). 1.01x the previous value.
